# rising-turtle/graph_slam

Hardware: AMD Instinct MI355X
Metric: Gauss-Newton iterations/s + final chi2 rel-err, 100k-pose SE3 graph (higher is better)
Workload: dtype f64; 1 GPU; 100k-pose / 1.00M-edge synthetic Manhattan-3D SE3 pose graph, 1xMI355X; poses=100000, edges=999944, parallelism=single GPU

## Files before the change

### graph_slam_amd/__init__.py

```python
import ctypes as C
import os

import numpy as np

_HERE = os.path.dirname(os.path.abspath(__file__))
LIB_PATH = os.environ.get("FGO_LIB", os.path.join(_HERE, "libfgo.so"))

FGO_TANGENT_G2O = 0
FGO_TANGENT_GTSAM = 1


class FgoConfig(C.Structure):
    _fields_ = [("device", C.c_int), ("verbose", C.c_int), ("ordering", C.c_int), ("nd_leaf", C.c_int), ("order_candidates", C.c_int),
                ("reserved", C.c_int * 11)]


class FgoStats(C.Structure):
    _fields_ = [("iterations", C.c_int), ("trials", C.c_int), ("terminated", C.c_int), ("structure_rebuilt", C.c_int),
                ("chi2_initial", C.c_double), ("chi2_final", C.c_double), ("lambda_final", C.c_double),
                ("t_symbolic", C.c_double), ("t_upload", C.c_double), ("t_total", C.c_double),
                ("ms_linearize", C.c_double), ("ms_factor", C.c_double), ("ms_solve", C.c_double), ("ms_update", C.c_double),
                ("n_free", C.c_int64), ("n_edges", C.c_int64), ("nnz_H_blocks", C.c_int64), ("nnz_L_blocks", C.c_int64),
                ("n_update_ops", C.c_int64), ("n_levels", C.c_int), ("n_tasks", C.c_int),
                ("bytes_factor", C.c_double), ("bytes_linearize", C.c_double), ("bytes_solve", C.c_double),
# ... 159 lines not shown
class MapRenderView(C.Structure):
    _fields_ = [(f, C.c_int64) for f in ("n_valid", "n_drawn", "n_pixels", "n_meas", "n_both", "n_agree", "n_closer", "n_through")]


class MapRenderResult(C.Structure):
    _fields_ = [("n_points", C.c_int64), ("n_nonfinite", C.c_int64), ("form", C.c_int), ("tile_rows", C.c_int)]


FGO_MAP_RENDER_TILES, FGO_MAP_RENDER_GLOBAL = 0, 1


ALLREDUCE_FN = C.CFUNCTYPE(C.c_int, C.c_void_p, C.c_void_p, C.c_int64)


def _load():
    if not os.path.exists(LIB_PATH):
        raise ImportError(
            "graph_slam_amd: %s is missing — build it with `python -m graph_slam_amd.build` "
            "(hipcc, gfx950).  There is no CPU fallback." % LIB_PATH)
    lib = C.CDLL(LIB_PATH)
    dp, ip, i64p = C.POINTER(C.c_double), C.POINTER(C.c_int), C.POINTER(C.c_int64)
    lib.fgo_create.restype = C.c_void_p
    lib.fgo_create.argtypes = [C.POINTER(FgoConfig)]
    lib.fgo_destroy.argtypes = [C.c_void_p]
    lib.fgo_last_error.restype = C.c_char_p
    lib.fgo_last_error.argtypes = [C.c_void_p]
    lib.fgo_version.restype = C.c_char_p
    lib.fgo_device_count.restype = C.c_int
    lib.fgo_add_pose.argtypes = [C.c_void_p, C.c_int64, dp, dp, C.c_int]
    lib.fgo_set_pose.argtypes = [C.c_void_p, C.c_int64, dp, dp]
    lib.fgo_get_pose.argtypes = [C.c_void_p, C.c_int64, dp]
    lib.fgo_has_pose.argtypes = [C.c_void_p, C.c_int64]
    lib.fgo_num_poses.restype = C.c_int64
    lib.fgo_num_poses.argtypes = [C.c_void_p]
    lib.fgo_num_edges.restype = C.c_int64
    lib.fgo_num_edges.argtypes = [C.c_void_p]
    lib.fgo_add_poses.argtypes = [C.c_void_p, C.c_int64, i64p, dp, C.POINTER(C.c_ubyte)]
    lib.fgo_get_poses.argtypes = [C.c_void_p, C.c_int64, i64p, dp]
    lib.fgo_add_edge_se3.argtypes = [C.c_void_p, C.c_int64, C.c_int64, dp, dp, dp, C.c_int]
    lib.fgo_add_edges_se3.argtypes = [C.c_void_p, C.c_int64, i64p, i64p, dp, dp, C.c_int]
    lib.fgo_optimize.argtypes = [C.c_void_p, C.c_int, C.POINTER(FgoStats)]
    lib.fgo_chi2.restype = C.c_double
    lib.fgo_chi2.argtypes = [C.c_void_p]
    lib.fgo_trace.argtypes = [C.c_void_p, dp, dp, C.c_int]
    lib.fgo_linearize.argtypes = [C.c_void_p, dp, dp, dp, i64p]
    lib.fgo_solve_step.argtypes = [C.c_void_p, C.c_double, dp]
    lib.fgo_bench_phase.argtypes = [C.c_void_p, C.c_int, C.c_int, dp]
    lib.fgo_get_stats.argtypes = [C.c_void_p, C.POINTER(FgoStats)]
    lib.fgo_synth_manhattan3d.restype = C.c_int64
    lib.fgo_synth_manhattan3d.argtypes = [C.c_int64, C.c_int, C.c_int, C.c_uint64, C.c_double, C.c_double,
                                          dp, dp, i64p, i64p, dp, dp, C.c_int64]
    lib.fgo_shard_range.argtypes = [C.c_int64, C.c_int, C.c_int, i64p, i64p]
    lib.fgo_add_prior_pose.argtypes = [C.c_void_p, C.c_int64, dp, dp, dp]
    lib.fgo_optimize_gtsam.argtypes = [C.c_void_p, C.c_int, C.POINTER(FgoStats)]
    lib.fgo_error.restype = C.c_double
    lib.fgo_isam2_update.argtypes = [C.c_void_p, C.c_double, C.POINTER(FgoStats)]
    lib.fgo_isam2_reset.argtypes = [C.c_void_p]
    lib.fgo_isam2_get_state.argtypes = [C.c_void_p, C.c_int64, dp, dp]
    lib.fgo_error.argtypes = [C.c_void_p]
    lib.fgo_marginal_cov.argtypes = [C.c_void_p, C.c_int64, dp]
    lib.fgo_set_shard.argtypes = [C.c_void_p, C.c_int, C.c_int]
    lib.fgo_set_allreduce.argtypes = [C.c_void_p, ALLREDUCE_FN, C.c_void_p]
    lib.fgo_isam2_reserve.argtypes = [C.c_void_p, C.c_int, C.c_int]
    lib.fgo_set_growth.argtypes = [C.c_void_p, C.c_int, C.c_int]
    lib.fgo_isam2_set_wildfire.argtypes = [C.c_void_p, C.c_double]
    lib.fgo_marginal_cov_many.argtypes = [C.c_void_p, C.c_int64, i64p, dp]
    lib.fgo_marginal_cov_all.restype = C.c_int64
    lib.fgo_marginal_cov_all.argtypes = [C.c_void_p, C.c_int64, i64p, dp]
    lib.fgo_marginal_cov_pairs.argtypes = [C.c_void_p, C.c_int64, i64p, i64p, dp]
    lib.fgo_debug_selinv_stats.argtypes = [C.c_void_p, dp]
    lib.fgo_debug_selinv_census.argtypes = [C.c_void_p, i64p]
    lib.fgo_gate_edges_se3.argtypes = [C.c_void_p, C.c_int64, i64p, i64p, dp, dp, C.c_int, dp, dp, dp]
    lib.fgo_edge_chi2_se3.argtypes = [C.c_void_p, C.c_int64, C.c_int64, dp]
    lib.fgo_debug_gate_stats.argtypes = [C.c_void_p, dp]
    lib.fgo_gate_plane_factors.argtypes = [C.c_void_p, C.c_int64, i64p, i64p, dp, dp, dp, dp, dp, dp, dp]
    lib.fgo_associate_planes.argtypes = [C.c_void_p, C.c_int64, C.c_int64, dp, dp, C.c_int64, i64p, C.c_double, C.c_double, i64p, dp, dp]
    lib.fgo_dist_unique_id.argtypes = [C.c_void_p]
    lib.fgo_dist_init_rccl.argtypes = [C.c_void_p, C.c_void_p]
    lib.fgo_debug_partition.argtypes = [C.c_int, C.c_int64, C.POINTER(C.c_int), C.POINTER(C.c_int), C.c_int, C.POINTER(C.c_int)]
    lib.fgo_debug_allreduce.argtypes = [C.c_void_p, dp, C.c_int64]
    lib.fgo_debug_read_system.argtypes = [C.c_void_p, dp, dp, dp]
    lib.fgo_debug_read_reduced.argtypes = [C.c_void_p, C.c_double, dp, dp, i64p]
    lib.fgo_debug_solve_fused.argtypes = [C.c_void_p, C.c_double, dp]
    lib.fgo_debug_launch_census.argtypes = [C.c_void_p, C.c_int, i64p, i64p, i64p, C.c_int, C.POINTER(C.c_int), C.POINTER(C.c_int), C.c_int,
                                            C.POINTER(C.c_int), C.c_char_p, C.c_int]
    lib.fgo_debug_isam_last.argtypes = [C.c_void_p] + [C.POINTER(C.c_int)] * 6 + [C.c_int,
                                        C.POINTER(C.c_int), C.c_char_p, C.c_char_p, C.c_int, C.POINTER(C.c_int), C.c_char_p, dp, C.c_int64]
    lib.fgo_debug_linearize_census.argtypes = [C.c_void_p, i64p]
    lib.fgo_imu_params_vn100.argtypes = [dp]
    lib.fgo_preint_reset.argtypes = [dp, dp]
    lib.fgo_preint_integrate.argtypes = [dp, dp, dp, dp, C.c_double]
    lib.fgo_preint_predict.argtypes = [dp] * 7
    lib.fgo_set_fixed.argtypes = [C.c_void_p, C.c_int64, C.c_int]
    lib.fgo_preint_information.argtypes = [dp, dp]
    lib.fgo_preint_batch.argtypes = [C.c_int, C.c_int64, C.POINTER(C.c_int64), dp, dp, C.c_double, dp, dp, dp]
    lib.fgo_two_view_params_default.restype = None
    lib.fgo_two_view_params_default.argtypes = [C.POINTER(TwoViewParams)]
    lib.fgo_two_view_ba_batch.argtypes = [C.c_int, C.c_int64, i64p, dp, dp, dp, dp, dp, dp, C.POINTER(TwoViewParams), dp, dp, dp, dp,
                                          C.POINTER(TwoViewResult)]
    lib.fgo_plane_check_params_default.restype = None
    lib.fgo_plane_check_params_default.argtypes = [C.POINTER(PlaneCheckParams)]
    lib.fgo_plane_check_vro_batch.argtypes = [C.c_int, C.c_int64, dp, dp, dp, i64p, dp, dp, i64p, dp, dp, C.POINTER(PlaneCheckParams),
                                              C.POINTER(PlaneCheckResult), i64p, dp, dp, dp, dp, dp]
    lib.fgo_chi2_quantile.restype = C.c_double
    lib.fgo_chi2_quantile.argtypes = [C.c_int, C.c_double]
    lib.fgo_imu_check_params_default.restype = None
    lib.fgo_imu_check_params_default.argtypes = [C.POINTER(ImuCheckParams)]
    lib.fgo_imu_check_vro_batch.argtypes = [C.c_int, C.c_int64, dp, dp, dp, C.c_int64, dp, i64p, dp, dp, C.POINTER(ImuCheckParams),
                                            C.POINTER(ImuCheckResult), dp, dp]
    lib.fgo_vro_params_default.restype = None
    lib.fgo_vro_params_default.argtypes = [C.POINTER(VroParams)]
    lib.fgo_vro_ransac_batch.argtypes = [C.c_int, C.c_int64, i64p, dp, dp, C.POINTER(VroParams), dp, dp, dp, C.POINTER(C.c_ubyte),
                                         C.POINTER(C.c_int32), C.POINTER(VroResult)]
    lib.fgo_debug_vro_waves.argtypes = [C.c_int]
    lib.fgo_debug_vro_kernel_ms.restype = C.c_double
    lib.fgo_debug_vro_kernel_ms.argtypes = []
    lib.fgo_plane_extract_params_default.restype = None
    lib.fgo_plane_extract_params_default.argtypes = [C.POINTER(PlaneExtractParams)]
    lib.fgo_plane_extract_batch.argtypes = [C.c_int, C.c_int64, C.c_int, C.c_int, C.POINTER(C.c_uint16), C.POINTER(PlaneExtractParams),
                                            C.POINTER(PlaneExtractResult), dp, dp, dp, C.POINTER(PlaneExtractPlane),
                                            C.POINTER(C.c_int8), C.POINTER(C.c_int32)]
    lib.fgo_debug_plane_extract_kernel_ms.restype = C.c_double
    lib.fgo_debug_plane_extract_kernel_ms.argtypes = []
    lib.fgo_plane_propagate_params_default.restype = None
    lib.fgo_plane_propagate_params_default.argtypes = [C.POINTER(PlanePropagateParams)]
    lib.fgo_plane_propagate_batch.argtypes = [C.c_int, C.c_int64, C.c_int, C.c_int, C.POINTER(C.c_uint16), C.POINTER(C.c_uint8),
                                              C.POINTER(C.c_int8), C.POINTER(C.c_int32), dp, dp, C.c_int64, i64p, i64p, dp, dp, dp,
                                              C.POINTER(PlanePropagateParams), C.POINTER(PlanePropagateResult), dp, dp, dp,
                                              C.POINTER(PlanePropagatePlane), C.POINTER(PlanePropagatePred), C.POINTER(C.c_int8)]
    lib.fgo_debug_plane_propagate_kernel_ms.restype = C.c_double
    lib.fgo_debug_plane_propagate_kernel_ms.argtypes = []
    lib.fgo_match_params_default.restype = None
    lib.fgo_match_params_default.argtypes = [C.POINTER(MatchParams)]
    i32p, u8p = C.POINTER(C.c_int32), C.POINTER(C.c_uint8)
    lib.fgo_match_features_batch.argtypes = [C.c_int, C.c_int64, i64p, u8p, dp, dp, C.c_int64, i64p, i64p, dp, u8p, C.POINTER(MatchParams),
                                             C.POINTER(MatchResult), i64p, i32p, i32p, i32p, u8p, i64p, i64p, i64p, dp, dp, dp, dp, i32p]
    lib.fgo_debug_match_kernel_ms.restype = C.c_double
    lib.fgo_debug_match_kernel_ms.argtypes = []
    lib.fgo_map_params_default.restype = None
    lib.fgo_map_params_default.argtypes = [C.POINTER(MapParams)]
    lib.fgo_map_fuse_batch.argtypes = [C.c_int, C.c_int64, C.c_int, C.c_int, C.POINTER(C.c_uint16), u8p, C.c_int, dp, dp, C.POINTER(MapParams),
                                       C.c_int64, C.POINTER(MapResult), dp, u8p, C.POINTER(C.c_int32), i64p, i64p, dp]
    lib.fgo_debug_map_fuse_kernel_ms.restype = C.c_double
    lib.fgo_debug_map_fuse_kernel_ms.argtypes = []
    lib.fgo_map_clean_params_default.restype = None
    lib.fgo_map_clean_params_default.argtypes = [C.POINTER(MapCleanParams)]
    lib.fgo_map_clean.argtypes = [C.c_int, C.c_int64, dp, C.POINTER(MapCleanParams), C.POINTER(MapCleanResult), C.POINTER(C.c_int32), u8p,
                                  C.POINTER(C.c_int32), i64p, dp]
    lib.fgo_debug_map_clean_kernel_ms.restype = C.c_double
    lib.fgo_debug_map_clean_kernel_ms.argtypes = []
    lib.fgo_map_normals_params_default.restype = None
    lib.fgo_map_normals_params_default.argtypes = [C.POINTER(MapNormalsParams)]
    lib.fgo_map_normals.argtypes = [C.c_int, C.c_int64, dp, C.POINTER(MapNormalsParams), C.POINTER(MapNormalsResult), dp, dp, dp, i32p, u8p,
                                    i32p, i64p, i64p]
    lib.fgo_debug_map_normals_kernel_ms.restype = C.c_double
    lib.fgo_debug_map_normals_kernel_ms.argtypes = []
    lib.fgo_map_render_params_default.restype = None
    lib.fgo_map_render_params_default.argtypes = [C.POINTER(MapRenderParams)]
    lib.fgo_map_render_batch.argtypes = [C.c_int, C.c_int64, dp, u8p, C.c_int, C.c_int64, dp, dp, dp, C.c_int, C.c_int,
                                         C.POINTER(MapRenderParams), C.POINTER(C.c_uint16), C.POINTER(MapRenderResult),
                                         C.POINTER(MapRenderView), i32p, i32p, u8p, dp]
    lib.fgo_debug_map_render_kernel_ms.restype = C.c_double
    lib.fgo_debug_map_render_kernel_ms.argtypes = []
    lib.fgo_add_vec3.argtypes = [C.c_void_p, C.c_int64, dp]
    lib.fgo_add_bias.argtypes = [C.c_void_p, C.c_int64, dp]
    lib.fgo_add_prior_vec3.argtypes = [C.c_void_p, C.c_int64, dp, C.c_double]
# ... 1047 lines not shown
        z = np.ascontiguousarray(z_abcd, np.float64); s = np.ascontiguousarray(cov_ut6, np.float64)
        self._chk(lib.fgo_add_plane_factor(self._h, pose_id, plane_id, _dp(z), _dp(s)))

    def add_point(self, pid, xyz):
        a = np.ascontiguousarray(xyz, np.float64)
        self._chk(lib.fgo_add_point3(self._h, pid, _dp(a)))

    def add_prior_point(self, pid, xyz, sigma):
        a = np.ascontiguousarray(xyz, np.float64)
        self._chk(lib.fgo_add_prior_point3(self._h, pid, _dp(a), sigma))

    def set_calibration(self, calib9, body_P_sensor7=None):
        c9 = [float(x) for x in calib9]
        b = None if body_P_sensor7 is None else _dp(np.ascontiguousarray(body_P_sensor7, np.float64))
        self._chk(lib.fgo_set_calib_ds2(self._h, *c9, b))

    def add_reproj(self, pose_id, point_id, uv, sigma=1.0):
        a = np.ascontiguousarray(uv, np.float64)
        self._chk(lib.fgo_add_reproj(self._h, pose_id, point_id, _dp(a), sigma))

    def optimize_gtsam(self, max_iters=100):
        st = FgoStats()
        rc = self._chk(lib.fgo_optimize_gtsam(self._h, max_iters, C.byref(st)))
        return rc, st

    def isam2_update(self, relinearize_threshold=0.1):
        st = FgoStats()
        self._chk(lib.fgo_isam2_update(self._h, relinearize_threshold, C.byref(st)))
        return st

    def isam2_set_wildfire(self, threshold):
        self._chk(lib.fgo_isam2_set_wildfire(self._h, threshold))

    def isam2_reserve(self, reserve_variables, window=0):
        self._chk(lib.fgo_isam2_reserve(self._h, reserve_variables, window))

    def set_growth(self, reserve_variables, window=0):
        self._chk(lib.fgo_set_growth(self._h, reserve_variables, window))

    def isam2_reset(self):
        self._chk(lib.fgo_isam2_reset(self._h))

    def isam2_state(self, pid):
        th = np.zeros(7); de = np.zeros(6)
        self._chk(lib.fgo_isam2_get_state(self._h, pid, _dp(th), _dp(de)))
        return th, de

    def error(self):
        v = lib.fgo_error(self._h)
        if v != v:
            raise FgoError("fgo_error failed: %s" % lib.fgo_last_error(self._h).decode())
        return v

    def trace(self, cap=256):
        a = np.zeros(cap); b = np.zeros(cap)
        m = self._chk(lib.fgo_trace(self._h, _dp(a), _dp(b), cap))
        return a[:m], b[:m]

    def linearize(self, dense=True):
        chi = C.c_double(); nf = C.c_int64()
        if not dense:
            self._chk(lib.fgo_linearize(self._h, C.byref(chi), None, None, C.byref(nf)))
            return chi.value, None, None
        self._chk(lib.fgo_linearize(self._h, C.byref(chi), None, None, C.byref(nf)))
        m = 6 * nf.value
        H = np.zeros((m, m)); b = np.zeros(m)
        self._chk(lib.fgo_linearize(self._h, C.byref(chi), _dp(H), _dp(b), C.byref(nf)))
        return chi.value, H, b

    def solve_step(self, lam):
        chi = C.c_double(); nf = C.c_int64()
        self._chk(lib.fgo_linearize(self._h, C.byref(chi), None, None, C.byref(nf)))
        d = np.zeros(6 * nf.value)
        self._chk(lib.fgo_solve_step(self._h, lam, _dp(d)))
        return d

    def solve_fused(self, lam):
        chi = C.c_double(); nf = C.c_int64()
        self._chk(lib.fgo_linearize(self._h, C.byref(chi), None, None, C.byref(nf)))
        d = np.zeros(6 * nf.value)
        self._chk(lib.fgo_debug_solve_fused(self._h, lam, _dp(d)))
        return d

    def launch_census(self, fused=True):
        ip = C.POINTER(C.c_int)
        names = C.create_string_buffer(4096)
        n = self._chk(lib.fgo_debug_launch_census(self._h, int(fused), None, None, None, 0, None, None, 0, None, names, len(names)))
        nl = int(self.stats().n_levels)
        la = np.zeros(n, np.int64); wg = np.zeros(n, np.int64); it = np.zeros(n, np.int64)
        lr = np.zeros(max(nl, 1), np.int32); ll = np.zeros(max(nl, 1), np.int32); ch = np.zeros(2, np.int32)
        self._chk(lib.fgo_debug_launch_census(self._h, int(fused), _i64p(la), _i64p(wg), _i64p(it), n, lr.ctypes.data_as(ip), ll.ctypes.data_as(ip), nl,
                                              ch.ctypes.data_as(ip), None, 0))
        keys = names.value.decode().split("\n")[:n]
        return dict(forms={k: (int(a), int(w), int(i)) for k, a, w, i in zip(keys, la, wg, it)}, level_riders=[int(v) for v in lr[:nl]],
                    level_long=[int(v) for v in ll[:nl]], chain_on=bool(ch[0]), chain_mode=int(ch[1]))

    def isam2_last(self):
        ip = C.POINTER(C.c_int)
        info = np.zeros(5, np.int32)
        n = self._chk(lib.fgo_debug_isam_last(self._h, info.ctypes.data_as(ip), None, None, None, None, None, 0, None, None, None, 0, None, None, None, 0))
        nl, nt = int(info[2]), int(info[3])
        lo = np.zeros(max(nl, 1), np.int32); hi = np.zeros(max(nl, 1), np.int32); cnt = np.zeros(max(nl, 1), np.int32)
        fw = np.zeros(max(nl, 1), np.int32); ft = np.zeros(max(nl, 1), np.int32)
        tl = np.zeros(max(nt, 1), np.int32); td = np.zeros(max(nt, 1), np.uint8); tr = np.zeros(max(nt, 1), np.uint8)
        vt = np.zeros(max(n, 1), np.int32); vc = np.zeros(max(n, 1), np.uint8); de = np.zeros((max(n, 1), 6))
        cp = lambda a: a.ctypes.data_as(C.c_char_p)
        self._chk(lib.fgo_debug_isam_last(self._h, info.ctypes.data_as(ip), lo.ctypes.data_as(ip), hi.ctypes.data_as(ip), cnt.ctypes.data_as(ip),
                                          fw.ctypes.data_as(ip), ft.ctypes.data_as(ip), nl,
                                          tl.ctypes.data_as(ip), cp(td), cp(tr), nt, vt.ctypes.data_as(ip), cp(vc), _dp(de), n))
        return dict(sweep=int(info[0]), cut=bool(info[1]), chain_low=int(info[4]), level_lo=lo[:nl], level_hi=hi[:nl], level_ntask=cnt[:nl], level_fwd=fw[:nl], level_fwtab=ft[:nl], task_level=tl[:nt],
                    task_dirty=td[:nt], task_run=tr[:nt], var_task=vt[:n], var_chg=vc[:n], delta=de[:n])

    LINEARIZE_CENSUS = ("n_hubs", "n_hub_vars", "n_hub_multi", "hub_deg", "hub_cap", "n_dup_groups", "n_dup_members", "n_priors",
                        "n_phantom", "imu_ncolor", "maskable", "structure_rebuilt")

    def linearize_census(self):
        out = np.zeros(12, np.int64)
        self._chk(lib.fgo_debug_linearize_census(self._h, _i64p(out)))
        return {k: int(v) for k, v in zip(self.LINEARIZE_CENSUS, out)}

    def bench_phase(self, phase, reps):
        ms = C.c_double()
        self._chk(lib.fgo_bench_phase(self._h, phase, reps, C.byref(ms)))
        return ms.value

    def stats(self):
        st = FgoStats()
        self._chk(lib.fgo_get_stats(self._h, C.byref(st)))
        return st
```

### graph_slam_amd/csrc/device_plan.hpp

```cpp
#pragma once
#include <hip/hip_runtime.h>
#include <stdint.h>
#include <vector>
#include "fgo_internal.hpp"

namespace fgo {

struct CamCalib {
  double fx, fy, s, u0, v0, k1, k2, p1, p2;
  double bps[7];
  double ad[36];
};
bool cam_calib_make(CamCalib &K, const double calib9[9], const double *body_P_sensor7);

struct ImuPayload {
  double dt;
  double dR[4];
  double dp[3], dv[3];
  double J_R_bg[9], J_p_ba[9], J_p_bg[9], J_v_ba[9], J_v_bg[9];
  double bhat[6];
  double info[225];
  double pad;
};
static_assert(sizeof(ImuPayload) == 288 * sizeof(double), "ImuPayload layout");

struct AccDesc { int t, a; long long o0, o1; };
struct LeafDesc { int task, c_begin, m, k0; long long base, obase; int nblk, nops; };
struct PanelDesc { int task, m, cols0, prow0, nrows, chunk0, nchunks, top; };
struct RowChunk { int pn, m, s0, R6, prow0, cols0, top, task; };
struct BwdChunk { int pn, m, row0, nrows; };
struct ChainItem { int pn, need; };

constexpr int NJMAX = (6 * PANEL_MAX + 15) / 16;
constexpr int NLT = NJMAX * (NJMAX - 1) / 2;
constexpr int NTILE = NLT + NJMAX;
constexpr int PTOP_TILE = 256;
static_assert(NTILE == NJMAX * (NJMAX + 1) / 2, "ptop: one slot per tile of the lower triangle, diagonal included");

struct PanelPlan {
  const PanelDesc *pdesc;
  const LeafDesc *leaf_desc, *leaf_lpt;
  const int *tri_order;
  const RowChunk *rchunks;
  const BwdChunk *bchunks;
  const ChainItem *bchain;
  unsigned *bchain_done;
  const int *task_panel, *panel_task;
  const int *ptri_blk;
  const int *prow_ptr, *prow_idx, *prow_blk;
  const int *pchunk_panel, *pchunk_row0, *pchunk_nrows, *panel_chunk0;
  const int64_t *row_mid;
  const int *fchunk_col;
  const int64_t *fchunk_e0;
  const int *pcol_fchunk0, *pcol_fchunkn;
  const int *rchunk_panel, *rchunk_s0;
  const int *rchunk_src;
  int rchunk_src0;
  const int *ptri_src, *prow_src;
  double *ptop;
  double *fpart;
  double *bpart;
};

struct RideItem;

constexpr int EDGE_REC = 32;
constexpr int HUB_DEG = 1024;
constexpr int HUB_SLICE = 512, HUB_MAX_SLICES = 64, HUB_MAX_VARS = 1024, HUB_PART = 42;

struct BaPlan {
  int n_lm;
  const unsigned char *lm_mine;
  int64_t n_obs;
  int n_tgt, n_cam;
  const int *lm_var;
  const int64_t *pt_ptr;
  const int *pt_obs;
  const double *pt_uvw;
  const int *pt_cam;
  const int64_t *lp_ptr;
  const double *lp_val;
  const double *obs_uvw;
  const int *obs_cam;
  const int *obs_col;
  const int *obs_lm;
  const int64_t *cam_ptr;
  const int *cam_col;
  int64_t o_first;
  int n_tgt_small;
  const int *tgt_list;
  int n_tgt_list;
  const int64_t *cam_t0;
  const int *cam_list;
  int n_cam_list;
  const int *tgt_blk;
  const int64_t *tgt_ptr;
  const int *op_a, *op_b;
  const int *op_lm;
  double *pt_val;
  double *Hinv, *zp;
};

struct DevPlan {
  PanelPlan pp;
  int64_t n_poses, n_edges;
  int64_t n_real;
  int64_t edge_stride;
  int64_t n_imu;
  const ImuPayload *imu;
  const int *imu_ids;
  const int *imu_slot;
  int64_t imu_fn;
  const int *imu_list;
  int imu_ncolor;
  const int *imu_color_ptr_h;
  double *imu_stash;
  double gravity[3];
  const int *var_kind;
  const int *edge_kind;
  CamCalib cam;
  int nb;
  int64_t n_hblocks;
  int lin_priors;
  int zero_offdiag;
  const int *pose_col;
  const int *edge_i, *edge_j;
  const double *ainv;
  const double *info;
  const int *edge_slot;
  const int *hub_list;
  const int *hub_slice;
  int n_hubs;
  int hub_deg;
  double *hub_part;
  const int *hubm;
  int n_hub_multi;
  const int64_t *he_ptr;
  const int *he;
  int64_t n_dup_groups;
  const int64_t *dup_ptr;
  const int64_t *dup_edges;
  const int *dup_slot;
  int64_t n_priors;
  const int64_t *prior_ptr;
  const int *prior_pose;
  const double *prior_minv;
  const double *prior_info;
  const int64_t *colptr;
  const int *rowidx;
  const int *asrc;
  int prof_tri;
  int zero_blk;
  const int64_t *op_ptr;
  const int64_t *op_mid;
  const int *op_a, *op_b;
  const int *acc_targets;
  const AccDesc *acc_desc;
  const int *g2_tgt;
  const int64_t *g2_ptr;
  const int *g2_b;
  const int *g2_a;
  const unsigned char *task_dirty;
  const int *acc_task;
  const int *g2_task;
  const int *tcol_task;
  BaPlan ba;
  const int *fwg_ci, *fwg_ch;
  const int *fwd_f0, *fwd_fn;
  const int *fsplit_ci;
  const RideItem *ride_items;
  int ride_xcd;
  const int64_t *acc_start;
  const int64_t *rowptr;
  const int *row_blk, *row_col;
  const int *task_ptr, *task_cols;
  double *partial;
  int dist;
  int top_col0;
  int64_t top_blk0;
  const int64_t *top_ext0;
  const int64_t *own_op0, *own_op1;
  const int64_t *top_row0;
  const int64_t *own_row0, *own_row1;
  const unsigned char *var_mine;
  int lambda_rank;
};

struct HostSchedule {
  int cus = 256;
  int n_levels = 0;
  int world = 1, rank = 0;
  std::vector<int> seg_group;
  int64_t n_top_blocks = 0;
  int n_top_cols = 0;
  std::vector<int> level_ptr;
  std::vector<int64_t> acc_ptr, acc_mid;
  std::vector<int> ride_ptr;
  std::vector<int64_t> g2_lvl;
  std::vector<int> level_maxcol;
  std::vector<int> level_maxrow;
  std::vector<int> level_maxtaskcols;
  std::vector<char> level_leaf;
  std::vector<int> level_leaf_maxblk, level_leaf_maxops;
  std::vector<char> level_panel;
  int rows_byc_level = 1 << 30;
  std::vector<int> level_pn0;
  std::vector<int> level_col_ptr;
  std::vector<int> fwg_ptr;
  std::vector<int> fsplit_ptr;
  std::vector<int> pchunk_ptr, fchunk_ptr, rchunk_ptr;
  int bchain_low = -1, bchain_n = 0;
};

void launch_linearize(const DevPlan &P, const double *poses, double *Hblk, double *bvec, double *scalar_out, hipStream_t s);
void launch_chi2(const DevPlan &P, const double *poses, double *scalar_out, hipStream_t s);
void launch_maxdiag(const DevPlan &P, const double *Hblk, double *scalar_out, hipStream_t s);
void launch_update(const DevPlan &P, const double *poses, double *cand, const double *x, const double *b,
                   const double *lambda_p, double *scalar_out, hipStream_t s);
enum { PHASE_ALL = 0, PHASE_DOMAIN = 1, PHASE_TOP = 2 };
struct PartialSweep {
  const int *t_lo, *t_hi;
  const int64_t *s0, *s1, *l0, *l1;
  const int *g0, *g1, *c0, *c1;
  const int *task_ptr;
};
enum LaunchForm {
  LF_ACC8 = 0, LF_ACC4, LF_ACC2, LF_ACC1,
  LF_ACC2_8, LF_ACC2_4, LF_ACC2_1,
  LF_FWD_COMBINE,
  LF_TRI16, LF_TRI8, LF_TRI1,
  LF_ROWS, LF_ROWS_BYC,
  LF_LEAF4,
  LF_FACT_1_2, LF_FACT_1_3, LF_FACT_4_3, LF_FACT_8_3, LF_FACT_16_2,
  LF_FWD1, LF_FWD4, LF_FWD16,
  LF_FWD_EXT, LF_FWD_TRI,
  LF_BWD_CHAIN, LF_BWD_FUSED, LF_BWD_EXT, LF_BWD_TRI,
  LF_BWD1, LF_BWD4, LF_BWD8,
  LF_COUNT
};
const char *launch_form_name(int form);
struct LaunchCensus {
  int64_t launches[LF_COUNT] = {}, workgroups[LF_COUNT] = {};
  int64_t items[LF_COUNT] = {};
  std::vector<int> level_riders, level_long;
  std::vector<int> level_fwd, level_fwtab;
  int chain_on = 0, chain_mode = 0;
  void add(int form, int64_t grid, int64_t n_items = -1) { ++launches[form]; workgroups[form] += grid; items[form] += n_items < 0 ? grid : n_items; }
};
LaunchForm select_acc(const HostSchedule &H, int l);
LaunchForm select_tri(const HostSchedule &H, int l);
LaunchForm select_rows(const HostSchedule &H, int l);
LaunchForm select_fact(const HostSchedule &H, int l);
LaunchForm select_fwd(const HostSchedule &H, int l);
LaunchForm select_bwd(const HostSchedule &H, int l);
void launch_factor(const DevPlan &P, const HostSchedule &H, const double *Hblk, double *Lv, const double *lambda_p,
                   int *fail_flag, hipStream_t s, const double *b = nullptr, double *x = nullptr, int phase = PHASE_ALL, const PartialSweep *ps = nullptr,
                   const double *b_full = nullptr, LaunchCensus *census = nullptr);
struct Wildfire { unsigned char *run, *chg; const unsigned char *dirty; const double *xprev; double thr; };
void launch_solve(const DevPlan &P, const HostSchedule &H, const double *Lv, const double *b, double *x, hipStream_t s,
                  bool fwd_done = false, int phase = PHASE_ALL, const Wildfire *wf = nullptr, LaunchCensus *census = nullptr);
void launch_mix_rhs(const DevPlan &P, const double *b, const double *ysaved, double *x, const unsigned char *col_dirty, hipStream_t s);
void launch_copy_vec(const double *src, double *dst, int64_t n, hipStream_t s);
void launch_mask_poses(const DevPlan &P, const double *poses, double *out, const int *pose_group, int rank, int world, hipStream_t s);
int linearize_blocks(const DevPlan &P);
void launch_reduce(const double *partial, int64_t n, double *out, int mode, hipStream_t s);
void prepare_device_kernels();
void launch_zero(double *p, int64_t n, hipStream_t s);
void launch_zero_flag(int *p, hipStream_t s);
void launch_pack_scalars(double *scal, const int *fail, hipStream_t s, double *host = nullptr);
void launch_fetch_scalar(double *dst, const double *src_host, hipStream_t s);
void launch_scatter_edges(const double *stage, int64_t n, int64_t e0, double *rec, hipStream_t s);
bool linearize_gtsam_maskable(const DevPlan &P);
void launch_linearize_gtsam_masked(const DevPlan &P, const double *poses, double *Hblk, double *bvec, double *scalar_out, hipStream_t s,
                                   const unsigned char *mask, double *chi_var);
void launch_linearize_gtsam(const DevPlan &P, const double *poses, double *Hblk, double *bvec, double *scalar_out, hipStream_t s,
                            double *ba_W = nullptr, double *ba_Hpp = nullptr, double *ba_bp = nullptr);
int ba_linearize_blocks(const DevPlan &P);
void launch_ba_linearize(const DevPlan &P, const double *vals, double *W, double *Hpp, double *bp, double *Hblk, double *bvec, double *chi_partial, hipStream_t s);
void launch_ba_reduce(const DevPlan &P, const double *W, const double *Hpp, const double *bp, const double *H, const double *b,
                      double *Hred, double *bred, const double *lambda_p, int *fail_flag, hipStream_t s);
void launch_ba_back(const DevPlan &P, const double *W, const double *bp, double *x, hipStream_t s);
void launch_chi2_gtsam(const DevPlan &P, const double *poses, double *scalar_out, hipStream_t s);
void launch_update_gtsam(const DevPlan &P, const double *poses, double *cand, const double *x, const double *b,
                         const double *lambda_p, double *scalar_out, hipStream_t s);
void launch_isam2_relin(const DevPlan &P, double *theta, double *delta, double thr, double *count_out, hipStream_t s, unsigned char *moved_out = nullptr);
void launch_isam2_estimate(const DevPlan &P, const double *theta, const double *x, double *delta, double *est, hipStream_t s,
                           unsigned char *moved_next = nullptr, double thr_next = 0);

struct SinvPlan {
  int nb;
  const int64_t *colptr;
  const int *task_ptr, *task_cols;
  const int64_t *sptr;
  const int *sidx;
  const double *U;
  double *Sig;
};
void launch_sinv_prep(const SinvPlan &Q, const double *Lv, double *U, hipStream_t s);
void launch_sinv_sweep(const SinvPlan &Q, const HostSchedule &H, hipStream_t s);
void launch_sinv_gather(const int64_t *enc, int64_t n, const double *Sig, double *out, hipStream_t s);
void launch_sinv_rows(const int *cols, int64_t n, const double *x, double *out, hipStream_t s, int64_t istride = 6, int64_t rstride = 1);

constexpr int64_t GATE_ZERO = -1, GATE_EXTRA0 = -2;
inline int64_t gate_extra_code(int64_t slot, bool transpose) { return GATE_EXTRA0 - ((slot << 1) | (transpose ? 1 : 0)); }
constexpr int GATE_REC = 28;
struct GatePlan {
  int64_t n;
  const int *va, *vb;
  const double *rec;
  const int64_t *enc;
  const double *Sig, *extra;
  double *out;
  int want_P;
};
void launch_gate(const GatePlan &A, const double *values, bool gtsam, bool with_cov, hipStream_t s);

constexpr int PGATE_REC = 10;
struct PlaneGatePlan {
  int64_t n;
  const int *vx, *vp;
  const double *rec;
  const int64_t *enc;
  const double *Sig, *extra;
  double *out;
  int want_P;
};
void launch_plane_gate(const PlaneGatePlan &A, const double *values, hipStream_t s);
void launch_plane_assoc(const double *gate_out, int64_t k, int64_t m, double d2_gate, double cos_min, bool want_matrix, double *res, hipStream_t s);

}
```

### graph_slam_amd/csrc/fgo_ctx.hpp

```cpp
#pragma once
#include <hip/hip_runtime.h>
#include <algorithm>
#include <atomic>
#include <chrono>
#include <cmath>
#include <cstdio>
#include <cstdlib>
#include <cstring>
#include <limits>
#include <map>
#include <mutex>
#include <new>
#include <stdexcept>
#include <string>
#include <unordered_map>
#include <vector>
#include "../../include/fgo.h"
#include "device_plan.hpp"
#include "fgo_internal.hpp"
#include "rccl_min.hpp"

namespace fgo {

template <class T>
struct DevBuf {
  T *p = nullptr;
  size_t n = 0, cap = 0;
  ~DevBuf() { release(); }
  void release() { if (p) { (void)hipFree(p); p = nullptr; n = 0; cap = 0; } }
  hipError_t alloc(size_t count) {
    if (p && count <= cap) { n = count; return hipSuccess; }
    const bool regrow = p != nullptr;
    release();
    cap = (count ? count : 1) + (regrow ? count / 4 : 0);
    const hipError_t e = hipMalloc((void **)&p, sizeof(T) * cap);
    if (e != hipSuccess) { p = nullptr; cap = 0; return e; }
    n = count;
    return hipSuccess;
  }
  template <class A>
  hipError_t upload(const std::vector<T, A> &h, hipStream_t s) {
    hipError_t e = alloc(h.size());
    if (e != hipSuccess) return e;
    if (h.empty()) return hipSuccess;
    return hipMemcpyAsync(p, h.data(), sizeof(T) * h.size(), hipMemcpyHostToDevice, s);
  }
  void swap(DevBuf &o) { std::swap(p, o.p); std::swap(n, o.n); std::swap(cap, o.cap); }
};

enum class LHolds { scratch, undamped, undamped_sigma, isam_step };

}

struct fgo_ctx {
  fgo_config cfg{};
  std::string err;
  std::unordered_map<int64_t, int> id2idx;
  std::vector<int64_t> ids;
  std::vector<double> poses;
  std::vector<unsigned char> fixed;
  std::vector<int> ei, ej;
  std::vector<double> meas, info;
  std::vector<int> torder;
  std::vector<int> prior_v;
  std::vector<double> prior_mean, prior_info;
  bool gtsam_mode = false;
  bool structure_dirty = true;
  bool host_poses_newer = true;
  bool dev_poses_newer = false;
  bool lin_valid = false;
  hipStream_t stream = nullptr;
  bool use_graph = true;
  fgo::Symbolic S;
  fgo::HostSchedule sched;
  fgo::DevPlan plan{};
  int64_t n_offdiag = 0;
  fgo::DevBuf<int> d_pose_col, d_edge_i, d_edge_j, d_edge_slot, d_he, d_dup_slot, d_rowidx, d_asrc, d_op_a, d_op_b,
      d_acc_targets, d_row_blk, d_row_col, d_task_ptr, d_task_cols, d_fail;
  fgo::DevBuf<int64_t> d_he_ptr, d_dup_ptr, d_dup_edges, d_colptr, d_op_ptr, d_op_mid, d_rowptr, d_g2_ptr;
  fgo::DevBuf<int> d_g2_tgt, d_g2_b, d_g2_a;
  fgo::DevBuf<fgo::RideItem> d_ride_items;
  fgo::DevBuf<int> d_fwg_ci, d_fwg_ch, d_fwd_f0, d_fwd_fn, d_fsplit_ci;
  fgo::DevBuf<int64_t> d_acc_start;
  fgo::DevBuf<double> d_ainv, d_partial, d_poses[2], d_H[2], d_b[2], d_x, d_L, d_scal;
  struct BaSchur {
    bool on = false;
    int n_lm = 0;
    fgo::DevBuf<unsigned char> d_lm_mine;
    fgo::DevBuf<int> d_lm_var, d_pt_obs, d_tgt_list, d_obs_cam, d_obs_col, d_obs_lm, d_cam_col, d_tgt_blk, d_op_a, d_op_b, d_op_lm, d_pt_cam;
    fgo::DevBuf<int64_t> d_pt_ptr, d_cam_ptr, d_tgt_ptr, d_lp_ptr, d_cam_t0;
    fgo::DevBuf<int> d_cam_list;
    fgo::DevBuf<double> d_obs_uvw, d_pt_uvw, d_lp_val, d_W[2], d_Hpp[2], d_bp[2], d_Hinv, d_zp, d_pt_val, d_Hred, d_bred;
  } ba;
  bool ba_disable = false;
  fgo::DevBuf<int> d_task_panel, d_panel_task, d_ptri_blk, d_prow_ptr, d_prow_idx, d_prow_blk, d_pchunk_panel, d_pchunk_row0,
      d_pchunk_nrows, d_panel_chunk0, d_fchunk_col, d_pcol_fchunk0, d_pcol_fchunkn;
  fgo::DevBuf<int64_t> d_row_mid, d_fchunk_e0;
  fgo::DevBuf<double> d_fpart, d_bpart, d_ptop, d_imu_stash;
  fgo::DevBuf<int> d_rchunk_panel, d_rchunk_s0, d_ptri_src, d_prow_src;
  fgo::DevBuf<int> d_hub_list, d_hub_slice, d_hubm;
  fgo::DevBuf<double> d_hub_part;
  fgo::DevBuf<fgo::PanelDesc> d_pdesc;
  fgo::DevBuf<int> d_tri_order, d_rchunk_src;
  fgo::DevBuf<fgo::LeafDesc> d_leaf_desc, d_leaf_lpt;
  fgo::DevBuf<fgo::AccDesc> d_acc_desc;
  fgo::DevBuf<fgo::RowChunk> d_rchunks;
  fgo::DevBuf<fgo::BwdChunk> d_bchunks;
  fgo::DevBuf<fgo::ChainItem> d_bchain;
  fgo::DevBuf<unsigned> d_bchain_done;
  fgo::DevBuf<int64_t> d_prior_ptr;
  fgo::DevBuf<int> d_prior_pose, d_var_kind, d_edge_kind;
  std::vector<int> var_kind;
  fgo::CamCalib cam{};
  bool cam_set = false;
  std::vector<int> imu_ids;
  std::vector<fgo::ImuPayload> imu_payload;
  double gravity[3] = {0.0, 0.0, 9.71};
  int shard_rank = 0, shard_world = 1;
  fgo_allreduce_fn ar_fn = nullptr;
  void *ar_user = nullptr;
  ncclComm_t rccl = nullptr;
  std::vector<int> pose_group;
  fgo::DevBuf<int> d_pose_group, d_imu_list;
  fgo::DevBuf<int64_t> d_top_ext0, d_own_op0, d_own_op1, d_top_row0, d_own_row0, d_own_row1;
  fgo::DevBuf<unsigned char> d_var_mine;
  fgo::DevBuf<double> d_status;
  fgo::DevBuf<double> d_gather;
  hipGraphExec_t dist_graph[2][2] = {{nullptr, nullptr}, {nullptr, nullptr}};
  double xgmi_bytes = 0;
  fgo::DevBuf<fgo::ImuPayload> d_imu;
  fgo::DevBuf<int> d_imu_ids, d_imu_slot;
  fgo::DevBuf<double> d_prior_minv, d_prior_info;
  int cur = 0;
  fgo::LHolds L_holds = fgo::LHolds::scratch;
  std::vector<int> h_pose_col;
  struct SelInv {
    bool lists = false;
    fgo::DevBuf<int64_t> d_sptr, d_enc;
    fgo::DevBuf<int> d_sidx;
    fgo::DevBuf<double> d_U, d_Sig, d_out;
    double t_build = 0, ms_factor = 0, ms_prep = 0, ms_sweep = 0;
    int64_t n_entries = 0, list_bytes = 0;
    int64_t n_fallback = 0;
    void release() {
      lists = false;
      d_sptr.release(); d_enc.release(); d_sidx.release(); d_U.release(); d_Sig.release(); d_out.release();
    }
  } sinv;
  struct Gate {
    fgo::DevBuf<int> d_v, d_cols;
    fgo::DevBuf<int64_t> d_enc;
    fgo::DevBuf<double> d_rec, d_extra, d_out, d_rhs, d_res;
    int64_t n_off = 0, n_groups = 0;
    double ms_kernel = 0, ms_solves = 0;
  } gate;
  fgo::DevBuf<double> d_theta, d_delta;
  int64_t isam_E_seen = 0, isam_NI_seen = 0, isam_NP_seen = 0;
  std::vector<int> col_task;
  fgo::DevBuf<double> d_y;
  fgo::DevBuf<unsigned char> d_moved, d_task_dirty, d_col_dirty, d_moved_next;
  unsigned char *h_flags = nullptr;
  fgo::DevBuf<unsigned char> d_lin_mask;
  fgo::DevBuf<double> d_chi_var;
  bool isam_H_valid = false;
  std::vector<int> isam_set_tasks, isam_set_cols;
  std::vector<int64_t> isam_set_aff;
  std::vector<int64_t> tk_s0, tk_s1, tk_l0, tk_l1;
  std::vector<int> tk_g0, tk_g1, tk_c0, tk_c1, task_level, lvl_lo, lvl_hi;
  bool tk_ok = false;
  int isam_last_sweep = 0;
  bool isam_last_cut = false;
  fgo::PartialSweep partial_sweep() const {
    return fgo::PartialSweep{lvl_lo.data(), lvl_hi.data(), tk_s0.data(), tk_s1.data(), tk_l0.data(), tk_l1.data(),
                             tk_g0.data(), tk_g1.data(), tk_c0.data(), tk_c1.data(), S.task_ptr.data()};
  }
  double wild_thr = 0;
  bool wild_valid = false;
  fgo::DevBuf<double> d_xprev;
  fgo::DevBuf<unsigned char> d_bwd_run, d_chg;
  bool isam_moved_valid = false;
  double isam_moved_thr = -1;
  int64_t isam_moved_nx = 0;
  size_t h_flags_cap = 0;
  fgo::DevBuf<int> d_acc_task, d_g2_task, d_tcol_task;
  int64_t isam_n = 0;
  bool isam_incremental = false;
// ... 101 lines not shown
```

### graph_slam_amd/csrc/fgo_inspect.cpp

```cpp
#include "fgo_ctx.hpp"

using namespace fgo;

extern "C" {

int fgo_debug_read_system(fgo_ctx *c, double *H, double *b, double *chi2) try {
  if (!c) return FGO_EINVAL;
  (void)hipSetDevice(c->cfg.device);
  ba_off(c);
  int rc = ensure_ready(c);
  if (rc) return rc;
  if (c->n_phantom > 0) return fail(c, FGO_ESTATE, "fgo_debug_read_system: the structure carries the growth reserve of the incremental mode (fgo_isam2_reset drops it)");
  hipStream_t s = c->stream;
  if (c->gtsam_mode) launch_linearize_gtsam(c->plan, c->d_poses[c->cur].p, c->d_H[c->cur].p, c->d_b[c->cur].p, c->d_scal.p + 0, s);
  else launch_linearize(c->plan, c->d_poses[c->cur].p, c->d_H[c->cur].p, c->d_b[c->cur].p, c->d_scal.p + 0, s);
  c->lin_valid = false;
  drop_undamped(c);
  if (H) HIPCHK(c, hipMemcpyAsync(H, c->d_H[c->cur].p, sizeof(double) * 36 * (size_t)c->plan.n_hblocks, hipMemcpyDeviceToHost, s));
  if (b) HIPCHK(c, hipMemcpyAsync(b, c->d_b[c->cur].p, sizeof(double) * 6 * (size_t)c->plan.nb, hipMemcpyDeviceToHost, s));
  if (chi2) HIPCHK(c, hipMemcpyAsync(chi2, c->d_scal.p, sizeof(double), hipMemcpyDeviceToHost, s));
  HIPCHK(c, hipStreamSynchronize(s));
  HIPCHK(c, hipGetLastError());
  return FGO_OK;
} FGO_CATCH_INT(c)
// ... 31 lines not shown
  HIPCHK(c, hipMemcpy(b.data(), db, sizeof(double) * b.size(), hipMemcpyDeviceToHost));
  HIPCHK(c, hipMemcpy(asrc.data(), c->d_asrc.p, sizeof(int) * asrc.size(), hipMemcpyDeviceToHost));
  const size_t m = (size_t)nreal * 6;
  if (H_dense) {
    std::memset(H_dense, 0, sizeof(double) * m * m);
    for (int k = 0; k < nb; ++k)
      for (int64_t t = c->S.colptr[k]; t < c->S.colptr[k + 1]; ++t) {
        if (asrc[t] < 0) continue;
        const int hr = c->S.perm[c->S.rowidx[t]], hc = c->S.perm[k];
        if (hr >= nreal || hc >= nreal) continue;
        const double *B = &H[(size_t)asrc[t] * 36];
        for (int r = 0; r < 6; ++r)
          for (int q = 0; q < 6; ++q) {
            H_dense[((size_t)hr * 6 + r) * m + (size_t)hc * 6 + q] = B[r * 6 + q];
            H_dense[((size_t)hc * 6 + q) * m + (size_t)hr * 6 + r] = B[r * 6 + q];
          }
      }
  }
  if (b_dense)
    for (int k = 0; k < nb; ++k) if (c->S.perm[k] < nreal) std::memcpy(b_dense + (size_t)c->S.perm[k] * 6, &b[(size_t)k * 6], 6 * sizeof(double));
  return FGO_OK;
}

int fgo_linearize(fgo_ctx *c, double *chi2_out, double *H_dense, double *b_dense, int64_t *n_free_out) try {
  if (!c) return FGO_EINVAL;
  (void)hipSetDevice(c->cfg.device);
  if (H_dense || b_dense) ba_off(c);
  int rc = ensure_ready(c);
  if (rc) return rc;
  rc = linearize_current(c, false);
  if (rc) return rc;
  if (chi2_out) *chi2_out = c->chi_cur;
  if (n_free_out) *n_free_out = (int64_t)c->plan.nb - c->n_phantom + (c->ba.on ? c->ba.n_lm : 0);
  if (!H_dense && !b_dense) return FGO_OK;
  return dense_from_blocks(c, c->d_H[c->cur].p, c->d_b[c->cur].p, H_dense, b_dense);
} FGO_CATCH_INT(c)

int fgo_debug_read_reduced(fgo_ctx *c, double lambda, double *H_dense, double *b_dense, int64_t *n_out) try {
  if (!c || !(lambda >= 0)) return FGO_EINVAL;
  (void)hipSetDevice(c->cfg.device);
  int rc = ensure_ready(c);
  if (rc) return rc;
  if (!c->ba.on) return fail(c, FGO_ESTATE, "fgo_debug_read_reduced: no landmarks are eliminated in this structure");
  rc = linearize_current(c, false);
  if (rc) return rc;
  if (n_out) *n_out = (int64_t)c->plan.nb - c->n_phantom;
  if (!H_dense && !b_dense) return FGO_OK;
  hipStream_t s = c->stream;
  HIPCHK(c, stage_lambda(c, lambda));
  launch_ba_reduce(c->plan, c->ba.d_W[c->cur].p, c->ba.d_Hpp[c->cur].p, c->ba.d_bp[c->cur].p, c->d_H[c->cur].p, c->d_b[c->cur].p,
                   c->ba.d_Hred.p, c->ba.d_bred.p, c->d_scal.p + 3, c->d_fail.p, s);
  HIPCHK(c, hipStreamSynchronize(s));
  HIPCHK(c, hipGetLastError());
  return dense_from_blocks(c, c->ba.d_Hred.p, c->ba.d_bred.p, H_dense, b_dense);
} FGO_CATCH_INT(c)

static int solve_once(fgo_ctx *c, double lambda, double *delta_out, bool fused, const char *who) {
  if (!c || !delta_out) return FGO_EINVAL;
  if (c->shard_world > 1) return fail(c, FGO_ESTATE, (std::string(who) + ": not available in distributed mode").c_str());
  (void)hipSetDevice(c->cfg.device);
  ba_off(c);
  int rc = ensure_ready(c);
  if (rc) return rc;
  if (!c->lin_valid) { rc = linearize_current(c, false); if (rc) return rc; }
  hipStream_t s = c->stream;
  claim_L(c);
  HIPCHK(c, stage_lambda(c, lambda));
  launch_factor(c->plan, c->sched, c->d_H[c->cur].p, c->d_L.p, c->d_scal.p + 3, c->d_fail.p, s, fused ? c->d_b[c->cur].p : nullptr, fused ? c->d_x.p : nullptr);
  launch_solve(c->plan, c->sched, c->d_L.p, c->d_b[c->cur].p, c->d_x.p, s, fused);
  const int nb = c->plan.nb;
  std::vector<double> x((size_t)nb * 6);
  HIPCHK(c, hipMemcpyAsync(x.data(), c->d_x.p, sizeof(double) * x.size(), hipMemcpyDeviceToHost, s));
  HIPCHK(c, hipMemcpyAsync(c->h_fail, c->d_fail.p, sizeof(int), hipMemcpyDeviceToHost, s));
  HIPCHK(c, hipStreamSynchronize(s));
  HIPCHK(c, hipGetLastError());
  for (int k = 0; k < nb; ++k)
    if (c->S.perm[k] < nb - c->n_phantom) std::memcpy(delta_out + (size_t)c->S.perm[k] * 6, &x[(size_t)k * 6], 6 * sizeof(double));
  if (*c->h_fail) return fail(c, FGO_ENUM, "block Cholesky: matrix not positive definite");
  return FGO_OK;
}
int fgo_solve_step(fgo_ctx *c, double lambda, double *delta_out) try { return solve_once(c, lambda, delta_out, false, "fgo_solve_step"); } FGO_CATCH_INT(c)
int fgo_debug_solve_fused(fgo_ctx *c, double lambda, double *delta_out) try { return solve_once(c, lambda, delta_out, true, "fgo_debug_solve_fused"); } FGO_CATCH_INT(c)

int fgo_debug_launch_census(fgo_ctx *c, int fused, int64_t *launches, int64_t *workgroups, int64_t *items, int form_cap, int *level_riders, int *level_long,
                            int level_cap, int *chain2, char *names, int names_cap) try {
  if (!c || form_cap < 0 || level_cap < 0 || names_cap < 0) return FGO_EINVAL;
  if (c->shard_world > 1) return fail(c, FGO_ESTATE, "fgo_debug_launch_census: not available in distributed mode");
  (void)hipSetDevice(c->cfg.device);
  if (fused != 2) ba_off(c);
  if (fused == 2 && (c->structure_dirty || c->isam_last_sweep == 0 || c->col_task.empty()))
    return fail(c, FGO_ESTATE, "fgo_debug_launch_census: the last fgo_isam2_update on this structure was not a partial sweep");
  int rc = ensure_ready(c);
  if (rc) return rc;
  LaunchCensus cz;
  double *const b = c->d_b[c->cur].p, *const x = c->d_x.p;
  if (!b || !x) return fail(c, FGO_ESTATE, "fgo_debug_launch_census: the right-hand side / solution buffers are not allocated");
  DevPlan plan = c->plan;
  PartialSweep ps{};
  if (fused == 2) { plan.task_dirty = c->d_task_dirty.p; if (c->isam_last_sweep == 2) ps = c->partial_sweep(); }
  launch_factor(plan, c->sched, c->d_H[c->cur].p, c->d_L.p, c->d_scal.p + 3, c->d_fail.p, c->stream, fused ? b : nullptr, fused ? x : nullptr, PHASE_ALL,
                fused == 2 && c->isam_last_sweep == 2 ? &ps : nullptr, nullptr, &cz);
  launch_solve(c->plan, c->sched, c->d_L.p, b, x, c->stream, fused != 0, PHASE_ALL, nullptr, &cz);
  for (int f = 0; f < std::min<int>(form_cap, LF_COUNT); ++f) {
    if (launches) launches[f] = cz.launches[f];
    if (workgroups) workgroups[f] = cz.workgroups[f];
    if (items) items[f] = cz.items[f];
  }
  for (int l = 0; l < std::min(level_cap, c->sched.n_levels); ++l) {
    if (level_riders) level_riders[l] = cz.level_riders[(size_t)l];
    if (level_long) level_long[l] = cz.level_long[(size_t)l];
  }
  if (chain2) { chain2[0] = cz.chain_on; chain2[1] = cz.chain_mode; }
  if (names && names_cap > 0) {
    std::string all;
    for (int f = 0; f < LF_COUNT; ++f) { all += launch_form_name(f); all += '\n'; }
    if ((int)all.size() + 1 > names_cap) return fail(c, FGO_EINVAL, "fgo_debug_launch_census: names buffer too small");
    std::memcpy(names, all.c_str(), all.size() + 1);
  }
  return LF_COUNT;
} FGO_CATCH_INT(c)

int fgo_debug_linearize_census(fgo_ctx *c, int64_t out[12]) try {
  if (!c || !out) return FGO_EINVAL;
  (void)hipSetDevice(c->cfg.device);
  int rc = ensure_ready(c);
  if (rc) return rc;
  const DevPlan &P = c->plan;
  out[0] = P.n_hubs; out[1] = c->n_hub_vars; out[2] = P.n_hub_multi; out[3] = P.hub_deg; out[4] = (int64_t)c->hub_entry_cap;
  out[5] = P.n_dup_groups; out[6] = c->n_dup_members;
  out[7] = P.n_priors; out[8] = c->n_phantom; out[9] = P.imu_ncolor;
  out[10] = c->gtsam_mode && linearize_gtsam_maskable(P) ? 1 : 0;
  out[11] = c->last_phase_rebuilt;
  return FGO_OK;
} FGO_CATCH_INT(c)

int fgo_debug_isam_last(fgo_ctx *c, int *info5, int *level_lo, int *level_hi, int *level_ntask, int *level_fwd, int *level_fwtab, int level_cap, int *task_level, unsigned char *task_dirty,
                        unsigned char *task_run, int task_cap, int *var_task, unsigned char *var_chg, double *var_delta, int64_t var_cap) try {
  if (!c || level_cap < 0 || task_cap < 0 || var_cap < 0) return FGO_EINVAL;
  (void)hipSetDevice(c->cfg.device);
  if (c->structure_dirty || c->col_task.empty() || !c->inc.valid || c->isam_n <= 0)
    return fail(c, FGO_ESTATE, "fgo_debug_isam_last: no fgo_isam2_update has run on the current structure");
  const int nl = c->sched.n_levels, ntask = (int)c->S.task_ptr.size() - 1, nb = c->plan.nb;
  const int64_t N = c->isam_n;
  if (info5) { info5[0] = c->isam_last_sweep; info5[1] = c->isam_last_cut ? 1 : 0; info5[2] = nl; info5[3] = ntask; info5[4] = c->sched.bchain_low; }
  const bool ranged = c->isam_last_sweep == 2;
  for (int l = 0; l < std::min(level_cap, nl); ++l) {
    if (level_lo) level_lo[l] = ranged ? c->lvl_lo[(size_t)l] : c->sched.level_ptr[l];
    if (level_hi) level_hi[l] = ranged ? c->lvl_hi[(size_t)l] : c->sched.level_ptr[l + 1] - 1;
    if (level_ntask) level_ntask[l] = c->sched.level_ptr[l + 1] - c->sched.level_ptr[l];
  }
  if ((level_fwd || level_fwtab) && level_cap > 0) {
    LaunchCensus cz;
    DevPlan plan = c->plan;
    PartialSweep ps{};
    if (c->isam_last_sweep != 0) plan.task_dirty = c->d_task_dirty.p;
    if (ranged) ps = c->partial_sweep();
    launch_factor(plan, c->sched, c->d_H[c->cur].p, c->d_L.p, c->d_scal.p + 3, c->d_fail.p, c->stream, c->d_b[c->cur].p, c->d_x.p, PHASE_ALL,
                  ranged ? &ps : nullptr, nullptr, &cz);
    for (int l = 0; l < std::min(level_cap, nl); ++l) {
      if (level_fwd) level_fwd[l] = cz.level_fwd[(size_t)l];
      if (level_fwtab) level_fwtab[l] = cz.level_fwtab[(size_t)l];
    }
  }
  const int nt = std::min(task_cap, ntask);
  if (task_level) for (int t = 0; t < nt; ++t) task_level[t] = c->task_level[(size_t)t];
  if (task_dirty) {
// ... 53 lines not shown
```

### graph_slam_amd/csrc/fgo_internal.hpp

```cpp
#pragma once
#include <cstdint>
#include <cstdlib>
#include <exception>
#include <thread>
#include <pthread.h>
#include <mutex>
#include <condition_variable>
#include <functional>
#include <atomic>
#include <algorithm>
#include <memory>
#include <string>
#include <unordered_map>
#include <vector>

namespace fgo {

template <class T>
struct NoInitAlloc : std::allocator<T> {
  template <class U> struct rebind { typedef NoInitAlloc<U> other; };
  NoInitAlloc() = default;
  template <class U> NoInitAlloc(const NoInitAlloc<U> &) {}
  template <class U> void construct(U *p) { ::new ((void *)p) U; }
  template <class U, class... A> void construct(U *p, A &&...a) { ::new ((void *)p) U(std::forward<A>(a)...); }
};
typedef std::vector<int, NoInitAlloc<int>> IntList;

inline int host_threads() {
  static const int nthreads = [] {
    const char *e = std::getenv("FGO_HOST_THREADS");
    int t = e ? std::atoi(e) : (int)std::min(32u, std::max(1u, std::thread::hardware_concurrency()));
    return std::max(1, t);
  }();
  return nthreads;
}
inline double tune(const char *key, double dflt) {
  static const std::unordered_map<std::string, double> *tab = [] {
    auto *m = new std::unordered_map<std::string, double>();
    if (const char *e = std::getenv("FGO_TUNE")) {
      std::string s(e);
      size_t i = 0;
      while (i < s.size()) {
        size_t j = s.find(',', i);
        if (j == std::string::npos) j = s.size();
        const std::string kv = s.substr(i, j - i);
        const size_t q = kv.find('=');
        if (q != std::string::npos && q > 0) (*m)[kv.substr(0, q)] = std::atof(kv.c_str() + q + 1);
        i = j + 1;
      }
    }
    return m;
  }();
  const auto it = tab->find(key);
  return it == tab->end() ? dflt : it->second;
}
class HostPool {
 public:
  static HostPool &get() {
    static std::once_flag once;
    std::call_once(once, [] { pthread_atfork(nullptr, nullptr, [] { instance().store(nullptr); }); });
    HostPool *p = instance().load();
    if (!p) {
      HostPool *fresh = new HostPool;
      if (instance().compare_exchange_strong(p, fresh)) p = fresh; else delete fresh;
    }
    return *p;
  }
  template <class F>
  bool run(int nworkers, F &&job) {
    std::unique_lock<std::mutex> own(busy_, std::try_to_lock);
    if (!own.owns_lock()) return false;
    ensure(nworkers);
    std::exception_ptr err;
    std::mutex err_m;
    auto guarded = [&](int w) {
      try { job(w); }
      catch (...) { std::lock_guard<std::mutex> g(err_m); if (!err) err = std::current_exception(); }
    };
    {
      std::lock_guard<std::mutex> lk(m_);
      job_ = guarded;
      active_ = std::min(nworkers, (int)th_.size());
      pending_ = active_;
      ++epoch_;
    }
    cv_.notify_all();
    guarded(-1);
    {
      std::unique_lock<std::mutex> lk(m_);
      done_.wait(lk, [&] { return pending_ == 0; });
      job_ = nullptr;
    }
    if (err) std::rethrow_exception(err);
    return true;
  }
 private:
  static std::atomic<HostPool *> &instance() { static std::atomic<HostPool *> p{nullptr}; return p; }
  void ensure(int n) {
    while ((int)th_.size() < n) {
      const int id = (int)th_.size();
      uint64_t seen;
      { std::lock_guard<std::mutex> lk(m_); seen = epoch_; }
      th_.emplace_back([this, id, seen]() mutable {
        for (;;) {
          std::function<void(int)> job;
          {
            std::unique_lock<std::mutex> lk(m_);
            cv_.wait(lk, [&] { return epoch_ != seen; });
            seen = epoch_;
            if (id >= active_) continue;
            job = job_;
          }
          job(id);
          { std::lock_guard<std::mutex> lk(m_); if (--pending_ == 0) done_.notify_all(); }
        }
      });
    }
  }
  std::mutex busy_, m_;
  std::condition_variable cv_, done_;
  std::vector<std::thread> th_;
  std::function<void(int)> job_;
  int active_ = 0, pending_ = 0;
  uint64_t epoch_ = 0;
};
template <class F>
inline void parallel_ranges(int n, int chunk, F &&fn) {
  const int nthreads = host_threads();
  const int nchunks = (n + chunk - 1) / chunk;
  const int nt = std::min(nthreads, nchunks);
  if (nt <= 1) { if (n > 0) fn(0, n); return; }
  std::atomic<int> next{0};
  auto worker = [&](int) {
    for (int c = next.fetch_add(1); c < nchunks; c = next.fetch_add(1)) fn(c * chunk, std::min(n, (c + 1) * chunk));
  };
  if (!HostPool::get().run(nt - 1, worker)) worker(-1);
}

// ... 97 lines not shown
```

### graph_slam_amd/csrc/kernels_factor.hip

```cpp
#include <hip/hip_runtime.h>
#include <mutex>
#include <vector>
#include <stdint.h>
#include "device_plan.hpp"
#include "fgo_internal.hpp"
#include "sweep_device.hpp"

namespace fgo {

typedef double d4_t __attribute__((ext_vector_type(4)));

__device__ __forceinline__ void row_update(Row6 &acc, const Row6 &a, const double *__restrict__ B) {
#pragma unroll
  for (int c = 0; c < 6; ++c) {
    const Row6 b = load_row(B + 6 * c);
    acc.v[c] -= a.v[0] * b.v[0] + a.v[1] * b.v[1] + a.v[2] * b.v[2] + a.v[3] * b.v[3] + a.v[4] * b.v[4] + a.v[5] * b.v[5];
  }
}
__device__ __forceinline__ Row6 load_A_row(const DevPlan &P, const double *__restrict__ Hblk, int64_t t, int r, double lambda) {
  const int a = P.asrc[t];
  Row6 x = {{0, 0, 0, 0, 0, 0}};
  if (a >= 0) {
    x = load_row(Hblk + 36 * (int64_t)a + 6 * r);
    if (a < P.nb) {
// ... 410 lines not shown
      if (q == b0) {
#pragma unroll
        for (int rr = 0; rr < 6; ++rr)
          if (rr == r) {
#pragma unroll
            for (int c = 0; c < 6; ++c) lq.v[c] = (c <= rr) ? Lk[rr * (rr + 1) / 2 + c] : 0.0;
          }
        if (x) {
#pragma unroll
          for (int rr = 0; rr < 6; ++rr) if (rr == r) yr[6 * ci + rr] = yk[rr];
        }
      } else {
        lq = trsm_row(load_row(Ls + 36 * q + 6 * r), Lk, invd);
        if (x) {
          const int i2 = lrow[q];
          if (i2 != 0xffff)
            xr[6 * i2 + r] -= lq.v[0] * yk[0] + lq.v[1] * yk[1] + lq.v[2] * yk[2] + lq.v[3] * yk[3] + lq.v[4] * yk[4] + lq.v[5] * yk[5];
        }
      }
      store_row(Ls + 36 * q + 6 * r, lq);
    }
    __syncthreads();
  }
  if (x) for (int i = threadIdx.x; i < 6 * m; i += NW * 64) x[6 * (int64_t)k0 + i] = yr[i];
  double2 *__restrict__ dst = reinterpret_cast<double2 *>(Lv + 36 * base);
  const double2 *__restrict__ src = reinterpret_cast<const double2 *>(Ls);
  for (int i = threadIdx.x; i < nblk * 18; i += NW * 64) dst[i] = src[i];
}

struct PairTab { unsigned char a[PM * (PM + 1) / 2], b[PM * (PM + 1) / 2]; };
constexpr PairTab make_pairs() {
  PairTab t{};
  int q = 0;
  for (int a = 0; a < PM; ++a)
    for (int b = 0; b <= a; ++b) { t.a[q] = (unsigned char)a; t.b[q] = (unsigned char)b; ++q; }
  return t;
}
__constant__ PairTab PAIRS = make_pairs();
#define PAIR_A PAIRS.a
#define PAIR_B PAIRS.b
#define TRI(rr, kk) ((((rr) * ((rr) + 1)) / 2 + (kk)) * 36)

template <bool FROM_LDS>
__device__ __forceinline__ Row6 trsm_row_blk(const Row6 &u, const double *__restrict__ L) {
  Row6 x;
#pragma unroll
  for (int c = 0; c < 6; ++c) {
    double s = u.v[c];
#pragma unroll
    for (int m = 0; m < 6; ++m) if (m < c) s -= x.v[m] * L[6 * c + m];
    x.v[c] = s / L[7 * c];
  }
  return x;
}

__device__ __forceinline__ void ride_items16(const DevPlan &P, const double *__restrict__ Hblk, double *__restrict__ Lv,
                                             const double *__restrict__ lambda_p, int item0, int nitems, int wg, double *__restrict__ smem) {
  const int lane = threadIdx.x & 63, wave = threadIdx.x >> 6;
  const int g = lane / 6, r = lane - 6 * g;
  const int part = wave >> 2, w4 = wave & 3;
  const int ii = RIDE_PER_WG * wg + part;
  const bool have = ii < nitems;
  const RideItem it = P.ride_items[item0 + (have ? ii : 0)];
  const bool run = have && (!P.task_dirty || P.task_dirty[it.task]);
  double *__restrict__ tile = smem + 360 * wave;
  if (run && lane < 60) {
    const int gid = w4 * 10 + g;
    Row6 acc = {{0, 0, 0, 0, 0, 0}};
    if (gid == 0 && it.first != 2) acc = it.first ? load_A_row(P, Hblk, it.t, r, *lambda_p) : load_row(Lv + 36 * (int64_t)it.t + 6 * r);
    apply_ops(P, Lv, acc, g, r, it.o0 + gid, it.o0 + it.n, 40, tile);
#pragma unroll
    for (int c = 0; c < 6; ++c) tile[6 * lane + c] = acc.v[c];
  }
  __syncthreads();
  const int tl = (int)threadIdx.x - 256 * part;
  if (run && tl < 36) {
    const double *pf = smem + 1440 * part;
    double sum = 0;
    for (int q = 0; q < 40; ++q) sum += pf[q * 36 + tl];
    Lv[36 * (int64_t)it.t + tl] = it.first == 2 ? -sum : sum;
  }
}

template <int NW>
__global__ __launch_bounds__(NW * 64) void k_panel_tri(DevPlan P, const double *__restrict__ Hblk, double *__restrict__ Lv, int pn0,
                                                    const double *__restrict__ lambda_p, int *__restrict__ fail_flag, int n_pn, int ride0, int n_ride, int n_real) {
  __shared__ __attribute__((aligned(16))) double T[PM * (PM + 1) / 2 * 36];
  if (NW == 16) {
    __shared__ __attribute__((aligned(16))) double ride_smem[NW == 16 ? 16 * 360 : 2];
    if ((int)blockIdx.x >= n_pn) {
      const int nwg = (int)gridDim.x - n_pn;
      ride_items16(P, Hblk, Lv, lambda_p, ride0, n_ride, P.ride_xcd ? xcd_contiguous((int)blockIdx.x - n_pn, nwg) : (int)blockIdx.x - n_pn, ride_smem);
      return;
    }
  }
  const long long t_begin = __builtin_readcyclecounter();
  if ((int)blockIdx.x >= n_real) return;
  const int pn = (NW == 8 && !P.task_dirty) ? P.pp.tri_order[pn0 + blockIdx.x] : pn0 + (int)blockIdx.x;
  const PanelDesc dsc = P.pp.pdesc[pn];
  if (!task_runs(P, dsc.task)) return;
  const int m = dsc.m;
  const int64_t tri0 = (int64_t)pn * (PM * PM);
  const int *__restrict__ tb = P.pp.ptri_blk + tri0;
  const int lane = threadIdx.x & 63, wave = threadIdx.x >> 6;
  const int g = lane / 6, r = lane - 6 * g;
  const bool lane_on = lane < 60;
  const int gid = wave * 10 + g;
  const double lambda = *lambda_p;
  const int npair = m * (m + 1) / 2;
  for (int gq = gid; lane_on && gq < npair; gq += NW * 10) {
    const int rr = PAIR_A[gq], kk = PAIR_B[gq];
    const int sc = P.pp.ptri_src[tri0 + rr * PM + kk];
    const double *base = sc >= 0 ? Lv + 36 * (int64_t)sc : (sc <= -2 ? Hblk + 36 * (int64_t)(-2 - sc) : Lv + 36 * (int64_t)P.zero_blk);
    Row6 x = load_row(base + 6 * r);
    if (sc <= -2 && rr == kk) {
#pragma unroll
      for (int c = 0; c < 6; ++c) x.v[c] += (c == r) ? lambda : 0.0;
    }
    store_row(&T[36 * gq + 6 * r], x);
  }
  __syncthreads();
  const int n = 6 * m, nJ = (n + 15) >> 4;
  long long *__restrict__ stamp = (P.prof_tri && n_real == 1 && m == PM) ? reinterpret_cast<long long *>(P.partial) : nullptr;
  if (stamp && threadIdx.x == 0) { stamp[0] = t_begin; stamp[1] = __builtin_readcyclecounter(); }
  if (wave == 0) {
    constexpr int HMAX = (PM + 9) / 10;
    for (int k = 0; k < m; ++k) {
      if (stamp && lane == 0) stamp[8 + 5 * k] = __builtin_readcyclecounter();
      Row6 acc[HMAX];
#pragma unroll
      for (int h = 0; h < HMAX; ++h) {
        const int rr = k + g + 10 * h;
        if (lane_on && rr < m) {
          acc[h] = load_row(&T[TRI(rr, k) + 6 * r]);
          if (k > 0) {
            const Row6 a = load_row(&T[TRI(rr, k - 1) + 6 * r]);
            const double *__restrict__ B = &T[TRI(k, k - 1)];
#pragma unroll
            for (int j = 0; j < 6; ++j)
#pragma unroll
              for (int c = 0; c < 6; ++c) acc[h].v[c] = fma(-a.v[j], B[6 * c + j], acc[h].v[c]);
          }
        }
      }
      if (lane_on && g == 0) store_row(&T[TRI(k, k) + 6 * r], acc[0]);
      __builtin_amdgcn_wave_barrier();
      if (stamp && lane == 0) stamp[8 + 5 * k + 1] = __builtin_readcyclecounter();
      double Lk[21], invd[6];
      const bool ok = chol6_lds(&T[TRI(k, k)], Lk, invd);
      if (!ok && lane == 0) atomicOr(fail_flag, 1);
      __builtin_amdgcn_wave_barrier();
      if (stamp && lane == 0) stamp[8 + 5 * k + 2] = __builtin_readcyclecounter() + (long long)(Lk[0] == 12345.678);
#pragma unroll
      for (int h = 0; h < HMAX; ++h) {
        const int rr = k + g + 10 * h;
        if (lane_on && rr < m) {
          Row6 x = trsm_row(acc[h], Lk, invd);
          if (rr == k) {
#pragma unroll
            for (int c = 0; c < 6; ++c) x.v[c] = (c <= r) ? x.v[c] : 0.0;
          }
          store_row(&T[TRI(rr, k) + 6 * r], x);
        }
      }
      if (stamp && lane == 0) stamp[8 + 5 * k + 3] = __builtin_readcyclecounter();
      __syncthreads();
      if (stamp && lane == 0) stamp[8 + 5 * k + 4] = __builtin_readcyclecounter();
    }
  } else {
    const int nn = lane & 15, q4 = lane >> 4;
    const int ntile = nJ * (nJ + 1) / 2;
    constexpr bool EXCL = NW >= 16;
    constexpr int NWORK = EXCL ? NW - NW / 4 : NW - 1;
    constexpr int NT = (NJMAX * (NJMAX + 1) / 2 + NWORK - 1) / NWORK;
    const bool idle = EXCL && (wave & 3) == 0;
    const int aw = EXCL ? wave - 1 - (wave >> 2) : wave - 1;
    d4_t C[NT];
    bool own[NT];
    int offA[NT], rrA[NT], offB[NT], rrB[NT], cj[NT], offE[NT][4], rrE[NT][4], tI[NT];
#pragma unroll
    for (int u = 0; u < NT; ++u) {
      const int p = aw + NWORK * u;
      own[u] = !idle && p < ntile;
      const int I = PAIR_A[own[u] ? p : 0], K = PAIR_B[own[u] ? p : 0];
      tI[u] = I;
      const int iA = 16 * I + nn, iB = 16 * K + nn;
      rrA[u] = iA < n ? iA / 6 : -1; offA[u] = TRI(iA / 6, 0) + (iA % 6) * 6;
      rrB[u] = iB < n ? iB / 6 : -1; offB[u] = TRI(iB / 6, 0) + (iB % 6) * 6;
      cj[u] = iB % 6;
      C[u] = d4_t{0.0, 0.0, 0.0, 0.0};
#pragma unroll
      for (int r4 = 0; r4 < 4; ++r4) {
        const int i = 16 * I + q4 + 4 * r4;
        rrE[u][r4] = i < n ? i / 6 : -1; offE[u][r4] = TRI(i / 6, 0) + (i % 6) * 6;
        if (own[u] && rrE[u][r4] >= 0 && rrB[u] >= 0 && rrE[u][r4] >= rrB[u]) C[u][r4] = T[offE[u][r4] + 36 * rrB[u] + cj[u]];
      }
    }
    for (int k = 0; k < m; ++k) {
      if (k > 0) {
#pragma unroll
        for (int u = 0; u < NT; ++u)
          if (own[u] && 16 * tI[u] + 15 >= 6 * k) {
#pragma unroll
            for (int kc = 0; kc < 2; ++kc) {
              const int c = 4 * kc + q4;
              double a = 0.0, b = 0.0;
              if (c < 6) {
                if (rrA[u] > k - 1) a = -T[offA[u] + (k - 1) * 36 + c];
                if (rrB[u] > k - 1) b = T[offB[u] + (k - 1) * 36 + c];
              }
              C[u] = __builtin_amdgcn_mfma_f64_16x16x4f64(a, b, C[u], 0, 0, 0);
            }
          }
#pragma unroll
        for (int u = 0; u < NT; ++u)
          if (own[u] && rrB[u] == k + 1) {
#pragma unroll
            for (int r4 = 0; r4 < 4; ++r4)
              if (rrE[u][r4] >= k + 1) T[offE[u][r4] + (k + 1) * 36 + cj[u]] = C[u][r4];
          }
      }
      __syncthreads();
    }
  }
  if (stamp && threadIdx.x == 0) stamp[2] = __builtin_readcyclecounter();
  auto Ls = [&](int i, int j) -> double {
    if (i >= n || j >= n) return (i == j) ? 1.0 : 0.0;
    const int rr = i / 6, kk = j / 6;
    if (rr < kk) return 0.0;
    return T[TRI(rr, kk) + (i - 6 * rr) * 6 + (j - 6 * kk)];
  };
  double *__restrict__ tp = P.pp.ptop + (int64_t)dsc.top * 256;
  __shared__ double Dt[NJMAX * 256];
  __shared__ double Dr[NW >= 16 ? NJMAX * 16 : 1];
  auto copy_out = [&](int gq0, int gstep, int e0, int estep) {
    for (int gq = gq0; lane_on && gq < npair; gq += gstep) {
      const int rr = PAIR_A[gq], kk = PAIR_B[gq];
      const int t = tb[rr * PM + kk];
      if (t >= 0) store_row(Lv + 36 * (int64_t)t + 6 * r, load_row(&T[36 * gq + 6 * r]));
    }
    for (int e = e0; e < (nJ * (nJ - 1) / 2) * 256; e += estep) {
      const int tile = e >> 8, kc = (e >> 6) & 3, l = e & 63;
      const int J = PAIR_A[tile] + 1, I = PAIR_B[tile];
      tp[e] = -Ls(16 * J + (l & 15), 16 * I + 4 * kc + (l >> 4));
    }
  };
  auto invert = [&]() {
    if ((int)threadIdx.x < 16 * nJ) {
      const int J = threadIdx.x >> 4, c = threadIdx.x & 15;
      double xc[16];
      const double *__restrict__ D = &Dt[J * 256];
      if (NW >= 16) {
        Dr[threadIdx.x] = 1.0 / D[c * 17];
        __builtin_amdgcn_wave_barrier();
      }
#pragma unroll
      for (int i = 0; i < 16; ++i) xc[i] = (i == c) ? 1.0 : 0.0;
#pragma unroll
      for (int i = 0; i < 16; ++i) {
        xc[i] *= NW >= 16 ? Dr[16 * J + i] : 1.0 / D[i * 17];
#pragma unroll
        for (int i2 = 0; i2 < 16; ++i2) if (i2 > i) xc[i2] = fma(-D[i2 * 16 + i], xc[i], xc[i2]);
      }
#pragma unroll
      for (int i = 0; i < 16; ++i) tp[(NLT + J) * 256 + 16 * c + i] = xc[i];
    }
  };
  if (NW < 16) copy_out(gid, NW * 10, (int)threadIdx.x, NW * 64);
  for (int e = threadIdx.x; e < nJ * 256; e += NW * 64) Dt[e] = Ls(16 * (e >> 8) + ((e >> 4) & 15), 16 * (e >> 8) + (e & 15));
  __syncthreads();
  if (NW < 16 || wave < 2) invert();
  else copy_out(gid - 20, (NW - 2) * 10, (int)threadIdx.x - 128, (NW - 2) * 64);
  if (stamp && threadIdx.x == 0) { stamp[3] = __builtin_readcyclecounter(); stamp[4] = wall_clock64(); }
}

constexpr int tri1_tile(int I, int K) { return I * (I + 1) / 2 + K; }
constexpr int TRI1_NR = 16 * NJMAX;
struct Tri1Ctx {
  const double *Hblk; double *Lv; double *tp; int64_t zero_blk;
  int m, n, nJ, lane, nn, q;
  double lambda;
  int rr[2], rho[2];
  bool rv[2], rpad[2];
};
__device__ __forceinline__ const double *tri1_src_row(const Tri1Ctx &X, const int *__restrict__ tsrc, int h, int k) {
  const int sc = tsrc[X.rr[h] * PM + k];
  const double *base = sc >= 0 ? X.Lv + 36 * (int64_t)sc : (sc <= -2 ? X.Hblk + 36 * (int64_t)(-2 - sc) : X.Lv + 36 * X.zero_blk);
  return base + 6 * X.rho[h];
}
__device__ __forceinline__ double tri1_bcast(double v, int l) {
  return __hiloint2double(__builtin_amdgcn_readlane(__double2hiint(v), l), __builtin_amdgcn_readlane(__double2loint(v), l));
}
constexpr int tri1_low(int i, int j) { return i * (i - 1) / 2 + j; }
__device__ __forceinline__ bool tri1_chol6(const double *__restrict__ sd, int lane, double (&Ls)[15], double (&invd)[6]) {
  Row6 row = load_row(&sd[6 * (lane < 5 ? lane : 5)]);
  bool ok = true;
#pragma unroll
  for (int j = 0; j < 6; ++j) {
    const double d = tri1_bcast(row.v[j], j);
    if (!(d > 0.0)) ok = false;
    const double inv = rsqrt_nr(d);
    invd[j] = inv;
    row.v[j] *= inv;
#pragma unroll
    for (int k = 0; k < 6; ++k)
      if (k > j) {
        const double lkj = tri1_bcast(row.v[j], k);
        Ls[tri1_low(k, j)] = lkj;
        row.v[k] = fma(-row.v[j], lkj, row.v[k]);
      }
  }
  return ok;
}
__device__ __forceinline__ Row6 tri1_trsm_row(const Row6 &u, const double (&Ls)[15], const double (&invd)[6]) {
  Row6 x, w = u;
#pragma unroll
  for (int c = 0; c < 6; ++c) {
    x.v[c] = w.v[c] * invd[c];
#pragma unroll
    for (int c2 = 0; c2 < 6; ++c2) if (c2 > c) w.v[c2] = fma(-x.v[c], Ls[tri1_low(c2, c)], w.v[c2]);
  }
  return x;
}
template <int K>
__device__ __forceinline__ void tri1_step(const Tri1Ctx &X, d4_t (&C)[NJMAX * (NJMAX + 1) / 2], Row6 (&sN)[2], bool &ok_all,
                                          double *__restrict__ W, double *__restrict__ Dt, double *__restrict__ D6,
                                          const int *__restrict__ tsrc, const int *__restrict__ tblk) {
  constexpr int c0 = 6 * K, K0 = c0 >> 4, K1 = (c0 + 5) >> 4;
  const int lane = X.lane, nn = X.nn, q = X.q;
  Row6 s[2] = {sN[0], sN[1]};
  if (K + 1 < X.m) {
#pragma unroll
    for (int h = 0; h < 2; ++h)
      if (X.rv[h] && X.rr[h] >= K + 1) sN[h] = load_row(tri1_src_row(X, tsrc, h, K + 1));
  }
#pragma unroll
  for (int h = 0; h < 2; ++h)
    if (X.rv[h] && X.rr[h] == K && tsrc[K * PM + K] <= -2) {
#pragma unroll
      for (int c = 0; c < 6; ++c) s[h].v[c] += (c == X.rho[h]) ? X.lambda : 0.0;
    }
  if constexpr (K > 0) {
#pragma unroll
    for (int I = 0; I < NJMAX; ++I)
#pragma unroll
      for (int Kt = 0; Kt < NJMAX; ++Kt)
        if ((Kt == K0 || Kt == K1) && Kt <= I && 16 * I + 15 >= c0 && I < X.nJ) {
          const int c = 16 * Kt + nn - c0;
          if (c >= 0 && c < 6) {
#pragma unroll
            for (int r4 = 0; r4 < 4; ++r4) W[(16 * I + q + 4 * r4) * 6 + c] = C[tri1_tile(I, Kt)][r4];
          }
        }
    __builtin_amdgcn_wave_barrier();
#pragma unroll
    for (int h = 0; h < 2; ++h)
// ... 80 lines not shown
  if (!task_runs(P, dsc.task)) return;
  Tri1Ctx X;
  X.Hblk = Hblk; X.Lv = Lv; X.zero_blk = P.zero_blk;
  X.m = dsc.m; X.n = 6 * dsc.m; X.nJ = (X.n + 15) >> 4;
  X.lane = threadIdx.x; X.nn = X.lane & 15; X.q = X.lane >> 4;
  X.lambda = *lambda_p;
  X.tp = P.pp.ptop + (int64_t)dsc.top * 256;
  const int lane = X.lane, n = X.n, nJ = X.nJ;
#pragma unroll
  for (int e = 0; e < PM * PM / 64; ++e) {
    tsrc[lane + 64 * e] = P.pp.ptri_src[(int64_t)pn * PM * PM + lane + 64 * e];
    tblk[lane + 64 * e] = P.pp.ptri_blk[(int64_t)pn * PM * PM + lane + 64 * e];
  }
  for (int e = lane; e < NJMAX * 256; e += 64) {
    const int i = (e >> 4) & 15, j = e & 15, J = e >> 8;
    Dt[e] = (i == j && 16 * J + i >= n) ? 1.0 : 0.0;
  }
#pragma unroll
  for (int h = 0; h < 2; ++h) {
    const int i = lane + 64 * h;
    X.rv[h] = i < n; X.rpad[h] = i < 16 * nJ && i < TRI1_NR;
    X.rr[h] = i / 6; X.rho[h] = i - 6 * X.rr[h];
  }
  __builtin_amdgcn_wave_barrier();
  d4_t C[NJMAX * (NJMAX + 1) / 2];
#pragma unroll
  for (int p = 0; p < NJMAX * (NJMAX + 1) / 2; ++p) C[p] = d4_t{0.0, 0.0, 0.0, 0.0};
  Row6 sN[2];
#pragma unroll
  for (int h = 0; h < 2; ++h) {
    sN[h] = Row6{{0, 0, 0, 0, 0, 0}};
    if (X.rv[h]) sN[h] = load_row(tri1_src_row(X, tsrc, h, 0));
  }
  bool ok_all = true;
  tri1_steps<0>(X, C, sN, ok_all, W, Dt, D6, tsrc, tblk);
  if (!ok_all && lane == 0) atomicOr(fail_flag, 1);
  __builtin_amdgcn_wave_barrier();
#pragma unroll
  for (int pass = 0; pass < (NJMAX + 3) / 4; ++pass) {
    const int J = 4 * pass + X.q, c = X.nn;
    if (J < nJ) {
      const double *__restrict__ D = &Dt[J * 256];
      double xc[16];
#pragma unroll
      for (int i = 0; i < 16; ++i) xc[i] = (i == c) ? 1.0 : 0.0;
#pragma unroll
      for (int i = 0; i < 16; ++i) {
        xc[i] *= 1.0 / D[i * 17];
#pragma unroll
        for (int i2 = 0; i2 < 16; ++i2) if (i2 > i) xc[i2] = fma(-D[i2 * 16 + i], xc[i], xc[i2]);
      }
#pragma unroll
      for (int i = 0; i < 16; ++i) X.tp[(NLT + J) * 256 + 16 * c + i] = xc[i];
    }
  }
}
__global__ __launch_bounds__(64) __attribute__((amdgpu_waves_per_eu(2, 2))) void k_panel_tri1(DevPlan P, const double *__restrict__ Hblk, double *__restrict__ Lv, int pn0,
                                                   const double *__restrict__ lambda_p, int *__restrict__ fail_flag) {
  tri1_body(P, Hblk, Lv, pn0, lambda_p, fail_flag);
}

__device__ __forceinline__ void ride_item_wave(const DevPlan &P, const double *__restrict__ Hblk, double *__restrict__ Lv,
                                               const double *__restrict__ lambda_p, int item, double *__restrict__ tile) {
  const RideItem it = P.ride_items[item];
  if (P.task_dirty && !P.task_dirty[it.task]) return;
  const int lane = threadIdx.x;
  const int g = lane / 6, r = lane - 6 * g;
  if (lane < 60) {
    Row6 acc = {{0, 0, 0, 0, 0, 0}};
    if (g == 0) acc = it.first ? load_A_row(P, Hblk, it.t, r, *lambda_p) : load_row(Lv + 36 * (int64_t)it.t + 6 * r);
    apply_ops(P, Lv, acc, g, r, it.o0 + g, it.o0 + it.n, 10, tile);
#pragma unroll
    for (int c = 0; c < 6; ++c) tile[6 * lane + c] = acc.v[c];
  }
  __builtin_amdgcn_wave_barrier();
  if (lane < 36) {
    double sum = 0;
#pragma unroll
    for (int q = 0; q < 10; ++q) sum += tile[q * 36 + lane];
    Lv[36 * (int64_t)it.t + lane] = sum;
  }
}

template <bool BYC = false>
__device__ __forceinline__ void panel_rows_body(const DevPlan &P, const double *__restrict__ Hblk, double *__restrict__ Lv, int chunk0,
                                                double *__restrict__ x, int n_chunks, const double *__restrict__ lambda_p, int ride0) {
  if ((int)blockIdx.x >= n_chunks) {
    __shared__ __attribute__((aligned(16))) double ride_tile[360];
    ride_item_wave(P, Hblk, Lv, lambda_p, ride0 + (int)blockIdx.x - n_chunks, ride_tile);
    return;
  }
  const int ci = chunk0 + xcd_contiguous(blockIdx.x, n_chunks);
  const RowChunk rc = P.pp.rchunks[ci];
  const int lane = threadIdx.x, nn = lane & 15, q = lane >> 4;
  int scq[4 * NJMAX];
  if constexpr (BYC) {
    const int *__restrict__ rsq = P.pp.rchunk_src + ((int64_t)(ci - P.pp.rchunk_src0) * 16 + nn) * PANEL_MAX;
#pragma unroll
    for (int e = 0; e < 4 * NJMAX; ++e) scq[e] = rsq[(16 * (e >> 2) + q + 4 * (e & 3)) / 6];
  }
  if (!task_runs(P, rc.task)) return;
  const int m = rc.m;
  const int n = 6 * m, nJ = (n + 15) >> 4;
  const int R6 = rc.R6;
  const int *__restrict__ cols = P.task_cols + rc.cols0;
  const double *__restrict__ tp = P.pp.ptop + (int64_t)rc.top * 256;
  constexpr int RS = ROW_SETS;
  constexpr int NE = 4 * NJMAX;
  int sc[RS][NE], rho[RS];
  int64_t rowoff[RS];
  bool valid[RS], rhs[RS];
#pragma unroll
  for (int u = 0; u < RS; ++u) {
    const int s = rc.s0 + 16 * u + nn;
    valid[u] = s < R6;
    rhs[u] = x != nullptr && s == R6;
    const int br = valid[u] ? s / 6 : 0;
    rho[u] = valid[u] ? s - 6 * br : 0;
    rowoff[u] = (int64_t)(rc.prow0 + br) * PM;
    const int *__restrict__ rs = P.pp.prow_src + rowoff[u];
#pragma unroll
    for (int e = 0; e < NE; ++e) {
      const int c = 16 * (e >> 2) + q + 4 * (e & 3);
      if constexpr (BYC) sc[u][e] = ((valid[u] || rhs[u]) && c < n) ? scq[e] : -1;
      else sc[u][e] = (valid[u] && c < n) ? rs[c / 6] : ((rhs[u] && c < n) ? cols[c / 6] : -1);
    }
  }
  d4_t Y[RS][NJMAX];
#pragma unroll
  for (int u = 0; u < RS; ++u)
#pragma unroll
    for (int e = 0; e < NE; ++e) {
      const int c = 16 * (e >> 2) + q + 4 * (e & 3);
      const int k = c / 6;
      const int code = sc[u][e];
      const double *base = code >= 0 ? Lv + 36 * (int64_t)code : (code <= -2 ? Hblk + 36 * (int64_t)(-2 - code) : Lv + 36 * (int64_t)P.zero_blk);
      if (rhs[u] && c < n) base = x + 6 * (int64_t)code;
      Y[u][e >> 2][e & 3] = base[6 * rho[u] + (c - 6 * k)];
    }
  auto load_tile_row = [&](int J, double (&A)[4 * NJMAX]) {
#pragma unroll
    for (int I = 0; I < NJMAX; ++I)
      if (I < J) {
#pragma unroll
        for (int kc = 0; kc < 4; ++kc) A[4 * I + kc] = tp[((J * (J - 1) / 2 + I) * 4 + kc) * 64 + lane];
      }
#pragma unroll
    for (int kc = 0; kc < 4; ++kc) A[4 * (NJMAX - 1) + kc] = tp[((NLT + J) * 4 + kc) * 64 + lane];
  };
  double Abuf[2][4 * NJMAX];
  load_tile_row(0, Abuf[0]);
#pragma unroll
  for (int J = 0; J < NJMAX; ++J)
    if (J < nJ) {
      double (&A)[4 * NJMAX] = Abuf[J & 1];
      if (J + 1 < nJ) load_tile_row(J + 1, Abuf[(J + 1) & 1]);
#pragma unroll
      for (int u = 0; u < RS; ++u) {
        d4_t acc = Y[u][J];
#pragma unroll
        for (int I = 0; I < J; ++I)
#pragma unroll
          for (int kc = 0; kc < 4; ++kc)
            acc = __builtin_amdgcn_mfma_f64_16x16x4f64(A[4 * I + kc], Y[u][I][kc], acc, 0, 0, 0);
        d4_t z = {0.0, 0.0, 0.0, 0.0};
#pragma unroll
        for (int kc = 0; kc < 4; ++kc) z = __builtin_amdgcn_mfma_f64_16x16x4f64(A[4 * (NJMAX - 1) + kc], acc[kc], z, 0, 0, 0);
        Y[u][J] = z;
      }
    }
#pragma unroll
  for (int u = 0; u < RS; ++u) {
    const int *__restrict__ rb = P.pp.prow_blk + rowoff[u];
    int tt[NE];
#pragma unroll
    for (int e = 0; e < NE; ++e) {
      const int c = 16 * (e >> 2) + q + 4 * (e & 3);
      tt[e] = (valid[u] && c < n) ? rb[c / 6] : -1;
    }
#pragma unroll
    for (int e = 0; e < NE; ++e) {
      const int c = 16 * (e >> 2) + q + 4 * (e & 3);
      if (tt[e] >= 0) Lv[36 * (int64_t)tt[e] + 6 * rho[u] + (c - 6 * (c / 6))] = Y[u][e >> 2][e & 3];
      if (rhs[u] && c < n) x[6 * (int64_t)sc[u][e] + (c - 6 * (c / 6))] = Y[u][e >> 2][e & 3];
    }
  }
}

__global__ __launch_bounds__(64) void k_panel_rows(DevPlan P, const double *__restrict__ Hblk, double *__restrict__ Lv, int chunk0,
                                                   double *__restrict__ x, int n_chunks, const double *__restrict__ lambda_p, int ride0) {
  panel_rows_body<false>(P, Hblk, Lv, chunk0, x, n_chunks, lambda_p, ride0);
}
__global__ __launch_bounds__(64) void k_panel_rows_byc(DevPlan P, const double *__restrict__ Hblk, double *__restrict__ Lv, int chunk0,
                                                       double *__restrict__ x, int n_chunks, const double *__restrict__ lambda_p, int ride0) {
  panel_rows_body<true>(P, Hblk, Lv, chunk0, x, n_chunks, lambda_p, ride0);
}

__global__ __launch_bounds__(64) void k_dist_acc(DevPlan P, const double *__restrict__ Hblk, double *__restrict__ Lv,
                                                 const double *__restrict__ lambda_p) {
  __shared__ __attribute__((aligned(16))) double tile[360];
  const int lane = threadIdx.x, g = lane / 6, r = lane - 6 * g;
  const int64_t q = (int64_t)blockIdx.x * 10 + g;
  const int64_t nq = (int64_t)P.zero_blk - P.top_blk0;
  const bool on = lane < 60 && q < nq;
  Row6 acc = {{0, 0, 0, 0, 0, 0}};
  const int64_t t = P.top_blk0 + (on ? q : 0);
  if (on) {
    const int a = P.asrc[t];
    if (a >= 0) {
      acc = load_row(Hblk + 36 * (int64_t)a + 6 * r);
      if (a < P.nb && P.lambda_rank) {
        const double lambda = *lambda_p;
#pragma unroll
        for (int c = 0; c < 6; ++c) acc.v[c] += (c == r) ? lambda : 0.0;
      }
    }
  }
  apply_ops(P, Lv, acc, g, r, on ? P.own_op0[q] : 0, on ? P.own_op1[q] : 0, 1, tile);
  if (on) store_row(Lv + 36 * t + 6 * r, acc);
}
__global__ __launch_bounds__(64) void k_dist_rhs(DevPlan P, const double *__restrict__ Lv, const double *__restrict__ bvec, double *__restrict__ x,
                                                 const double *__restrict__ bfull) {
  __shared__ double sred[60];
  const int kq = blockIdx.x, k = P.top_col0 + kq;
  const int lane = threadIdx.x, g = lane / 6, r = lane - 6 * g;
  const int64_t e0 = P.own_row0[kq], e1 = P.own_row1[kq];
  double acc = 0;
  if (lane < 60) {
    for (int64_t e = e0 + g; e < e1; e += 40) {
      int bi[4], ci[4];
#pragma unroll
      for (int q = 0; q < 4; ++q) {
        const int64_t ee = e + 10 * q;
        const bool in = ee < e1;
        bi[q] = in ? P.row_blk[ee] : P.zero_blk;
        ci[q] = in ? P.row_col[ee] : 0;
      }
      Row6 l[4], y[4];
#pragma unroll
      for (int q = 0; q < 4; ++q) { l[q] = load_row(Lv + 36 * (int64_t)bi[q] + 6 * r); y[q] = load_row(x + 6 * (int64_t)ci[q]); }
#pragma unroll
      for (int q = 0; q < 4; ++q)
        acc += l[q].v[0] * y[q].v[0] + l[q].v[1] * y[q].v[1] + l[q].v[2] * y[q].v[2] + l[q].v[3] * y[q].v[3] + l[q].v[4] * y[q].v[4] + l[q].v[5] * y[q].v[5];
    }
    sred[lane] = acc;
  }
  __syncthreads();
  if (lane < 6) {
    double sv = P.lambda_rank ? bvec[6 * (int64_t)k + lane] : (bfull ? bvec[6 * (int64_t)k + lane] - bfull[6 * (int64_t)k + lane] : 0.0);
    for (int q = 0; q < 10; ++q) sv -= sred[q * 6 + lane];
    x[6 * (int64_t)k + lane] = sv;
  }
}

void prepare_device_kernels() {
  static std::mutex mu;
  static std::vector<char> done;
  int dev = 0;
  if (hipGetDevice(&dev) != hipSuccess || dev < 0) return;
  std::lock_guard<std::mutex> lock(mu);
  if ((int)done.size() <= dev) done.resize(dev + 1, 0);
  if (done[dev]) return;
  (void)hipFuncSetAttribute(reinterpret_cast<const void *>(&k_chol_leaf<4>), hipFuncAttributeMaxDynamicSharedMemorySize, 160 * 1024);
  done[dev] = 1;
}

struct LevelRange {
  bool nothing_dirty;
  int64_t sf, sn;
  int64_t lf; int n_long;
  int n_acc_wg;
  bool fw_table;
  int col0, n_fwd_wg;
  int64_t g2f; int n_g2;
  int t0, nt, pn0;
  int c0, nc;
};
static LevelRange level_range(const HostSchedule &H, const PartialSweep *ps, int l, bool fwd) {
  LevelRange R{};
  const int64_t a0 = H.acc_ptr[l], am = H.acc_mid[l], a1 = H.acc_ptr[l + 1];
  const int t0f = H.level_ptr[l], ntf = H.level_ptr[l + 1] - t0f;
  const bool panel = H.level_panel[l];
  const int n_g2_full = H.g2_lvl.empty() ? 0 : (int)(H.g2_lvl[l + 1] - H.g2_lvl[l]);
  const int64_t g2_first = H.g2_lvl.empty() ? 0 : H.g2_lvl[l];
  R.fw_table = H.fwg_ptr[l + 1] - H.fwg_ptr[l] != H.level_col_ptr[l + 1] - H.level_col_ptr[l];
  R.col0 = R.fw_table ? -1 - H.fwg_ptr[l] : H.level_col_ptr[l];
  const int n_fwd_full = (fwd && panel) ? (R.fw_table ? H.fwg_ptr[l + 1] - H.fwg_ptr[l] : H.level_col_ptr[l + 1] - H.level_col_ptr[l]) : 0;
  const int ta = ps ? ps->t_lo[l] : 0, tb = ps ? ps->t_hi[l] : -1;
  R.nothing_dirty = ps && tb < ta;
  if (!ps) {
    R.sf = a0; R.sn = am - a0;
    R.lf = am; R.n_long = (int)(a1 - am);
    R.n_fwd_wg = n_fwd_full;
    R.g2f = g2_first; R.n_g2 = n_g2_full;
    R.t0 = t0f; R.nt = ntf;
    if (panel) { R.c0 = H.rchunk_ptr[l]; R.nc = H.rchunk_ptr[l + 1] - H.rchunk_ptr[l]; }
  } else if (R.nothing_dirty) {
    R.sf = a0; R.sn = 0;
    R.lf = am; R.n_long = 0;
    R.n_fwd_wg = 0;
    R.g2f = g2_first; R.n_g2 = 0;
    R.t0 = t0f; R.nt = 0;
    if (panel) { R.c0 = H.rchunk_ptr[l]; R.nc = 0; }
  } else {
    R.sf = ps->s0[ta]; R.sn = ps->s1[tb] - ps->s0[ta];
    R.lf = ps->l0[ta]; R.n_long = (int)(ps->l1[tb] - ps->l0[ta]);
    R.n_fwd_wg = n_fwd_full;
    if (n_fwd_full > 0 && !R.fw_table) { R.col0 = ps->task_ptr[ta]; R.n_fwd_wg = ps->task_ptr[tb + 1] - ps->task_ptr[ta]; }
    if (n_g2_full == 0) { R.g2f = g2_first; R.n_g2 = 0; }
    else { R.g2f = ps->g0[ta]; R.n_g2 = ps->g1[tb] - ps->g0[ta]; }
    R.t0 = ta; R.nt = tb - ta + 1;
    if (panel) { R.c0 = ps->c0[ta]; R.nc = ps->c1[tb] - ps->c0[ta]; }
  }
  R.n_acc_wg = R.n_long > 0 ? (cdiv(R.sn, 10) + 7) & ~7 : cdiv(R.sn, 10);
  R.pn0 = panel ? H.level_pn0[l] + (R.t0 - t0f) : 0;
  return R;
}

void launch_factor(const DevPlan &P, const HostSchedule &H, const double *Hblk, double *Lv, const double *lambda_p,
                   int *fail_flag, hipStream_t s, const double *b, double *x, int phase, const PartialSweep *ps, const double *b_full, LaunchCensus *cz) {
  if (x && phase != PHASE_TOP && !P.task_dirty && !cz) launch_copy_vec(b, x, (int64_t)P.top_col0 * 6, s);
  if (cz) { cz->level_riders.assign((size_t)H.n_levels, 0); cz->level_long.assign((size_t)H.n_levels, 0); cz->level_fwd.assign((size_t)H.n_levels, 0); cz->level_fwtab.assign((size_t)H.n_levels, 0); }
  for (int l = 0; l < H.n_levels; ++l) {
    if (!seg_runs(H, l, phase)) continue;
    const LevelRange R = level_range(H, ps, l, x != nullptr);
    const int grid = R.n_acc_wg + R.n_long + R.n_fwd_wg, grid2 = R.n_g2 + R.n_fwd_wg;
    if (cz) { cz->level_fwd[(size_t)l] = R.n_fwd_wg; cz->level_fwtab[(size_t)l] = (R.fw_table && R.n_fwd_wg > 0) ? 1 : 0; }
    const LaunchForm acc = select_acc(H, l);
    const bool acc_g2 = acc == LF_ACC2_8 || acc == LF_ACC2_4 || acc == LF_ACC2_1;
    if (cz && !acc_g2 && grid > 0) cz->level_long[(size_t)l] = R.n_long;
    if (acc_g2 ? grid2 > 0 : grid > 0)
      switch (acc) {
        case LF_ACC2_8: FGO_LAUNCH_N(cz, acc, grid2, R.n_g2, k_chol_acc2<8>, dim3(grid2), dim3(512), 0, s, P, Hblk, Lv, Lv, R.g2f, R.n_g2, lambda_p, x, R.col0); break;
        case LF_ACC2_4: FGO_LAUNCH_N(cz, acc, grid2, R.n_g2, k_chol_acc2<4>, dim3(grid2), dim3(256), 0, s, P, Hblk, Lv, Lv, R.g2f, R.n_g2, lambda_p, x, R.col0); break;
        case LF_ACC2_1: FGO_LAUNCH_N(cz, acc, grid2, R.n_g2, k_chol_acc2<1>, dim3(grid2), dim3(64), 0, s, P, Hblk, Lv, Lv, R.g2f, R.n_g2, lambda_p, x, R.col0); break;
        case LF_ACC8: FGO_LAUNCH_N(cz, acc, grid, R.sn + R.n_long, k_chol_acc<8>, dim3(grid), dim3(512), 0, s, P, Hblk, Lv, R.sf, R.sn, lambda_p, x, R.n_acc_wg, R.col0, R.n_long, R.lf); break;
        case LF_ACC4: FGO_LAUNCH_N(cz, acc, grid, R.sn + R.n_long, k_chol_acc<4>, dim3(grid), dim3(256), 0, s, P, Hblk, Lv, R.sf, R.sn, lambda_p, x, R.n_acc_wg, R.col0, R.n_long, R.lf); break;
        case LF_ACC2: FGO_LAUNCH_N(cz, acc, grid, R.sn + R.n_long, k_chol_acc<2>, dim3(grid), dim3(128), 0, s, P, Hblk, Lv, R.sf, R.sn, lambda_p, x, R.n_acc_wg, R.col0, R.n_long, R.lf); break;
        default: FGO_LAUNCH_N(cz, LF_ACC1, grid, R.sn + R.n_long, k_chol_acc<1>, dim3(grid), dim3(64), 0, s, P, Hblk, Lv, R.sf, R.sn, lambda_p, x, R.n_acc_wg, R.col0, R.n_long, R.lf); break;
      }
    if (x && H.level_panel[l] && !H.fsplit_ptr.empty() && H.fsplit_ptr[l + 1] > H.fsplit_ptr[l] && !R.nothing_dirty)
      FGO_LAUNCH(cz, LF_FWD_COMBINE, H.fsplit_ptr[l + 1] - H.fsplit_ptr[l], k_fwd_combine, dim3(H.fsplit_ptr[l + 1] - H.fsplit_ptr[l]), dim3(64), 0, s, P, x, H.fsplit_ptr[l]);
    const int t0 = R.t0, nt = R.nt;
    if (H.level_panel[l]) {
      switch (select_tri(H, l)) {
        case LF_TRI1:
          if (nt > 0) FGO_LAUNCH(cz, LF_TRI1, nt, k_panel_tri1, dim3(nt), dim3(64), 0, s, P, Hblk, Lv, R.pn0, lambda_p, fail_flag);
          break;
        case LF_TRI8:
          if (nt > 0) FGO_LAUNCH(cz, LF_TRI8, nt, (k_panel_tri<8>), dim3(nt), dim3(8 * 64), 0, s, P, Hblk, Lv, R.pn0, lambda_p, fail_flag, nt, 0, 0, nt);
          break;
        default: {
          constexpr int TRI_NW = 16;
          const int r0 = H.ride_ptr.empty() ? 0 : H.ride_ptr[2 * l], nr = H.ride_ptr.empty() ? 0 : H.ride_ptr[2 * l + 1] - r0;
          const int ntp = (nr > 0 && P.ride_xcd) ? (nt + 7) & ~7 : nt;
          if (ntp + nr > 0) {
            if (cz) cz->level_riders[(size_t)l] += nr;
            FGO_LAUNCH(cz, LF_TRI16, ntp + (nr + RIDE_PER_WG - 1) / RIDE_PER_WG, (k_panel_tri<TRI_NW>), dim3(ntp + (nr + RIDE_PER_WG - 1) / RIDE_PER_WG), dim3(TRI_NW * 64), 0, s, P, Hblk, Lv, R.pn0, lambda_p, fail_flag, ntp, r0, nr, nt);
          }
        }
      }
      const int q0 = H.ride_ptr.empty() ? 0 : H.ride_ptr[2 * l + 1], nq = H.ride_ptr.empty() ? 0 : H.ride_ptr[2 * l + 2] - q0;
      if (R.nc + nq > 0) {
        if (cz) cz->level_riders[(size_t)l] += nq;
        if (select_rows(H, l) == LF_ROWS_BYC) FGO_LAUNCH(cz, LF_ROWS_BYC, R.nc + nq, k_panel_rows_byc, dim3(R.nc + nq), dim3(64), 0, s, P, Hblk, Lv, R.c0, x, R.nc, lambda_p, q0);
        else FGO_LAUNCH(cz, LF_ROWS, R.nc + nq, k_panel_rows, dim3(R.nc + nq), dim3(64), 0, s, P, Hblk, Lv, R.c0, x, R.nc, lambda_p, q0);
      }
      continue;
    }
    if (nt <= 0) continue;
    const LaunchForm fact = select_fact(H, l);
    switch (fact) {
      case LF_LEAF4: {
        const int lb = H.level_leaf_maxblk[l], lc = H.level_maxtaskcols[l];
        const size_t lds = ((size_t)lb + 1) * 36 * sizeof(double) + (size_t)12 * lc * sizeof(double) + ((size_t)lb + 2 + lc + 2) * sizeof(int) +
                           ((size_t)lb + 2) * sizeof(unsigned short) + (size_t)H.level_leaf_maxops[l] * sizeof(unsigned);
        FGO_LAUNCH(cz, LF_LEAF4, nt, (k_chol_leaf<4>), dim3(nt), dim3(256), lds, s, P, Hblk, Lv, t0, lambda_p, fail_flag, lb, lc, x);
        break;
      }
      case LF_FACT_1_2: FGO_LAUNCH(cz, fact, nt, (k_chol_fact<1, 2>), dim3(nt), dim3(64), 0, s, P, Hblk, Lv, t0, lambda_p, fail_flag); break;
      case LF_FACT_1_3: FGO_LAUNCH(cz, fact, nt, (k_chol_fact<1, 3>), dim3(nt), dim3(64), 0, s, P, Hblk, Lv, t0, lambda_p, fail_flag); break;
      case LF_FACT_4_3: FGO_LAUNCH(cz, fact, nt, (k_chol_fact<4, 3>), dim3(nt), dim3(256), 0, s, P, Hblk, Lv, t0, lambda_p, fail_flag); break;
      case LF_FACT_8_3: FGO_LAUNCH(cz, fact, nt, (k_chol_fact<8, 3>), dim3(nt), dim3(512), 0, s, P, Hblk, Lv, t0, lambda_p, fail_flag); break;
      default: FGO_LAUNCH(cz, LF_FACT_16_2, nt, (k_chol_fact<16, 2>), dim3(nt), dim3(1024), 0, s, P, Hblk, Lv, t0, lambda_p, fail_flag); break;
    }
    if (x && fact != LF_LEAF4) launch_fwd_level(P, H, Lv, x, l, s, cz);
  }
  if (phase == PHASE_DOMAIN && !cz) {
    if (H.n_top_blocks > 0) hipLaunchKernelGGL(k_dist_acc, dim3(cdiv(H.n_top_blocks, 10)), dim3(64), 0, s, P, Hblk, Lv, lambda_p);
    if (x && H.n_top_cols > 0) hipLaunchKernelGGL(k_dist_rhs, dim3(H.n_top_cols), dim3(64), 0, s, P, Lv, b, x, b_full);
  }
}

}
```

### graph_slam_amd/csrc/launch_select.cpp

```cpp
#include "device_plan.hpp"
#include "fgo_internal.hpp"

namespace fgo {

const char *launch_form_name(int form) {
  static const char *const names[LF_COUNT] = {
    "k_chol_acc<8>", "k_chol_acc<4>", "k_chol_acc<2>", "k_chol_acc<1>", "k_chol_acc2<8>", "k_chol_acc2<4>", "k_chol_acc2<1>", "k_fwd_combine",
    "k_panel_tri<16>", "k_panel_tri<8>", "k_panel_tri1", "k_panel_rows", "k_panel_rows_byc", "k_chol_leaf<4>",
    "k_chol_fact<1,2>", "k_chol_fact<1,3>", "k_chol_fact<4,3>", "k_chol_fact<8,3>", "k_chol_fact<16,2>",
    "k_solve_fwd<1>", "k_solve_fwd<4>", "k_solve_fwd<16>", "k_fwd_ext", "k_fwd_tri",
    "k_bwd_chain", "k_bwd_fused", "k_bwd_ext", "k_bwd_tri", "k_solve_bwd<1>", "k_solve_bwd<4>", "k_solve_bwd<8>"};
  return form >= 0 && form < LF_COUNT ? names[form] : "?";
}
LaunchForm select_acc(const HostSchedule &H, int l) {
  const int n_g2_full = H.g2_lvl.empty() ? 0 : (int)(H.g2_lvl[l + 1] - H.g2_lvl[l]);
  if (n_g2_full > 0) {
    static const int g2_narrow = (int)tune("acc2_narrow", 400);
    static const int g2_mid = (int)tune("acc2_mid", 6000);
    return n_g2_full <= g2_narrow ? LF_ACC2_8 : n_g2_full <= g2_mid ? LF_ACC2_4 : LF_ACC2_1;
  }
  const int64_t n = H.acc_ptr[l + 1] - H.acc_ptr[l];
  static const int64_t narrow_max = (int64_t)tune("acc_narrow", 4000);
  static const int64_t acc_wide2 = (int64_t)tune("acc_wide2", 60000);
  static const int64_t acc_mid2 = (int64_t)tune("acc_mid2", 15000);
  static const int acc_wide_split = (int)tune("acc_wide_split", 1);
  if (n <= narrow_max) return LF_ACC8;
  if (n > acc_wide2) return acc_wide_split == 1 ? LF_ACC1 : LF_ACC2;
  return n > acc_mid2 ? LF_ACC2 : LF_ACC4;
}
LaunchForm select_tri(const HostSchedule &H, int l) {
  const int ntf = H.level_ptr[l + 1] - H.level_ptr[l];
  const int tri_wide = tri_wide_panels(H.cus);
  static const int tri1_on = (int)tune("tri1", 1);
  const int tri1_min = (int)tune("tri1_min", 3 * H.cus);
  if (tri1_on && ntf > tri_wide && ntf >= tri1_min) return LF_TRI1;
  return ntf > tri_wide ? LF_TRI8 : LF_TRI16;
}
LaunchForm select_rows(const HostSchedule &H, int l) { return l >= H.rows_byc_level ? LF_ROWS_BYC : LF_ROWS; }
LaunchForm select_fact(const HostSchedule &H, int l) {
  if (!H.level_leaf.empty() && H.level_leaf[l]) return LF_LEAF4;
  static const int h1_2 = (int)tune("fact_h1_2", 20), h1_3 = (int)tune("fact_h1_3", 30), h4 = (int)tune("fact_h4", 120), h8 = (int)tune("fact_h8", 240);
  const bool single = H.level_maxtaskcols[l] == 1;
  const int h = H.level_maxcol[l];
  if (single && h <= h1_2) return LF_FACT_1_2;
  if (single && h <= h1_3) return LF_FACT_1_3;
  return h <= h4 ? LF_FACT_4_3 : h <= h8 ? LF_FACT_8_3 : LF_FACT_16_2;
}
LaunchForm select_fwd(const HostSchedule &H, int l) {
  static const int h1 = (int)tune("fwd_h1", 40), h4 = (int)tune("fwd_h4", 160);
  if (H.level_maxtaskcols[l] == 1 && H.level_maxrow[l] <= h1) return LF_FWD1;
  return H.level_maxrow[l] <= h4 ? LF_FWD4 : LF_FWD16;
}
LaunchForm select_bwd(const HostSchedule &H, int l) {
  if (H.level_panel[l]) {
    static const int bwd_fused_max = (int)tune("bwd_fused", 256);
    return H.level_ptr[l + 1] - H.level_ptr[l] <= bwd_fused_max ? LF_BWD_FUSED : LF_BWD_EXT;
  }
  static const int h1 = (int)tune("bwd_h1", 20), h4 = (int)tune("bwd_h4", 80);
  if (H.level_maxtaskcols[l] == 1 && H.level_maxcol[l] <= h1) return LF_BWD1;
  return H.level_maxcol[l] <= h4 ? LF_BWD4 : LF_BWD8;
}

}
```

### graph_slam_amd/csrc/structure_upload.cpp

```cpp
#include "structure_build.hpp"

namespace fgo {
namespace {

int upload_factor_side(fgo_ctx *c, const VarIndex &V, const Ordering &O, const HostTables &T, HubPlan &hubs, size_t &hub_cap) {
  hipStream_t s = c->stream;
  HIPCHK(c, c->d_pose_col.upload(T.pose_col, s));
  if (V.R > 0) {
    HIPCHK(c, c->d_edge_i.alloc((size_t)T.E_cap)); HIPCHK(c, c->d_edge_j.alloc((size_t)T.E_cap)); HIPCHK(c, c->d_edge_slot.alloc((size_t)T.E_cap));
    HIPCHK(c, c->d_edge_kind.alloc((size_t)T.E_cap)); HIPCHK(c, c->d_he.alloc((size_t)2 * T.E_cap));
    HIPCHK(c, c->d_imu.alloc((size_t)T.NI_cap)); HIPCHK(c, c->d_imu_ids.alloc((size_t)6 * T.NI_cap)); HIPCHK(c, c->d_imu_slot.alloc((size_t)15 * T.NI_cap));
    HIPCHK(c, c->d_imu_list.alloc((size_t)T.NI_cap));
  }
  HIPCHK(c, c->d_edge_i.upload(c->ei, s));
  HIPCHK(c, c->d_edge_j.upload(c->ej, s));
  HIPCHK(c, c->d_edge_slot.upload(T.edge_slot, s));
  HIPCHK(c, c->d_he_ptr.upload(T.he_ptr, s));
  plan_hubs(T.he_ptr, V.NX, 0, hubs);
  hub_cap = hubs.var.size() + (V.R > 0 ? 256 : 0);
  { const int rc = upload_hubs(c, hubs, hub_cap); if (rc) return rc; }
  HIPCHK(c, c->d_he.upload(T.he, s));
  HIPCHK(c, c->d_dup_ptr.upload(T.dup_ptr, s));
  HIPCHK(c, c->d_dup_edges.upload(T.dup_edges, s));
  HIPCHK(c, c->d_dup_slot.upload(T.dup_slot, s));
  c->n_dup_members = (int64_t)T.dup_edges.size();
  HIPCHK(c, c->d_ainv.upload(T.erec, s));
  { const int rc = upload_priors(c, V.NX, T.var_mine); if (rc) return rc; }
  HIPCHK(c, c->d_imu.upload(c->imu_payload, s));
  HIPCHK(c, c->d_imu_ids.upload(c->imu_ids, s));
  HIPCHK(c, c->d_imu_slot.upload(T.imu_slot, s));
  {
    std::vector<int> vk(c->var_kind);
    vk.resize((size_t)V.NX, 5);
    HIPCHK(c, c->d_var_kind.upload(vk, s));
    HIPCHK(c, hipStreamSynchronize(s));
  }
  HIPCHK(c, c->d_edge_kind.upload(c->torder, s));
  HIPCHK(c, c->d_imu_list.upload(T.imu_list, s));
  HIPCHK(c, c->d_pose_group.upload(c->pose_group, s));
  HIPCHK(c, c->d_var_mine.upload(T.var_mine, s));
  HIPCHK(c, c->d_top_ext0.upload(T.top_ext0, s));
  HIPCHK(c, c->d_own_op0.upload(T.own_op0, s));
  HIPCHK(c, c->d_own_op1.upload(T.own_op1, s));
  HIPCHK(c, c->d_top_row0.upload(T.top_row0, s));
  HIPCHK(c, c->d_own_row0.upload(T.own_row0, s));
  HIPCHK(c, c->d_own_row1.upload(T.own_row1, s));
  if (O.dist) HIPCHK(c, c->d_gather.alloc(std::max<size_t>((size_t)V.N * 8, 64)));
  return FGO_OK;
}

int host_schedule(fgo_ctx *c, const Ordering &O) {
  hipStream_t s = c->stream;
  const Symbolic &S = c->S;
  DevPlan &P = c->plan;
  c->sched.world = O.world; c->sched.rank = O.rank; c->sched.seg_group = S.seg_group;
  c->sched.n_top_blocks = S.nnzL - O.top_blk0; c->sched.n_top_cols = O.nb - O.top_col0;
  c->sched.ride_ptr = S.ride_items.empty() ? std::vector<int>() : S.ride_ptr;
  c->sched.g2_lvl = S.g2_lvl;
  if (S.g2_ptr.size() <= 1) c->sched.g2_lvl.clear();
  c->sched.level_panel = S.level_panel; c->sched.pchunk_ptr = S.pchunk_ptr; c->sched.fchunk_ptr = S.fchunk_ptr; c->sched.rchunk_ptr = S.rchunk_ptr;
  if (std::getenv("FGO_NO_PANELS")) std::fill(c->sched.level_panel.begin(), c->sched.level_panel.end(), 0);
  c->sched.level_leaf = S.level_leaf; c->sched.level_leaf_maxblk = S.level_leaf_maxblk; c->sched.level_leaf_maxops = S.level_leaf_maxops;
  if (tune("no_leaf", 0) != 0) std::fill(c->sched.level_leaf.begin(), c->sched.level_leaf.end(), 0);
  c->sched.n_levels = (int)S.level_ptr.size() - 1;
  c->sched.level_ptr = S.level_ptr;
  c->sched.acc_ptr = S.acc_ptr; c->sched.acc_mid = S.acc_mid;
  c->sched.level_pn0.assign(c->sched.n_levels, 0);
  for (int l = 0; l < c->sched.n_levels; ++l)
    if (S.level_panel[l]) {
      c->sched.level_pn0[l] = S.task_panel[S.level_ptr[l]];
      for (int t = S.level_ptr[l]; t < S.level_ptr[l + 1]; ++t)
        if (S.task_panel[t] != c->sched.level_pn0[l] + (t - S.level_ptr[l])) return fail(c, FGO_EINVAL, "internal: panel ids of a level are not consecutive");
    }
  c->sched.level_col_ptr.resize(c->sched.n_levels + 1);
  for (int l = 0; l <= c->sched.n_levels; ++l) c->sched.level_col_ptr[l] = S.task_ptr[S.level_ptr[l]];
  {
    static const int fwd_split = (int)tune("fwd_split", 32);
    std::vector<int> fwg_ci, fwg_ch, fsplit, f0v((size_t)O.nb, 0), fnv((size_t)O.nb, 1);
    c->sched.fwg_ptr.assign((size_t)c->sched.n_levels + 1, 0);
    c->sched.fsplit_ptr.assign((size_t)c->sched.n_levels + 1, 0);
    for (int l = 0; l < c->sched.n_levels; ++l) {
      if (S.level_panel[l])
        for (int t = S.level_ptr[l]; t < S.level_ptr[l + 1]; ++t) {
          const int pn = S.task_panel[t], m = S.task_ptr[t + 1] - S.task_ptr[t];
          for (int q = 0; q < m; ++q) {
            const int ci = S.task_ptr[t] + q;
            const int f0 = S.pcol_fchunk0[S.col_off(pn) + q], fn = S.pcol_fchunkn[S.col_off(pn) + q];
            if (fn <= 1 || O.dist || !fwd_split || fn < fwd_split) { fwg_ci.push_back(ci); fwg_ch.push_back(-1); continue; }
            f0v[(size_t)ci] = f0; fnv[(size_t)ci] = fn; fsplit.push_back(ci);
            for (int x = 0; x < fn; ++x) { fwg_ci.push_back(ci); fwg_ch.push_back(f0 + x); }
          }
        }
      c->sched.fwg_ptr[(size_t)l + 1] = (int)fwg_ci.size();
      c->sched.fsplit_ptr[(size_t)l + 1] = (int)fsplit.size();
    }
    HIPCHK(c, c->d_fwg_ci.upload(fwg_ci, s)); HIPCHK(c, c->d_fwg_ch.upload(fwg_ch, s));
    HIPCHK(c, c->d_fwd_f0.upload(f0v, s)); HIPCHK(c, c->d_fwd_fn.upload(fnv, s));
    HIPCHK(c, c->d_fsplit_ci.upload(fsplit, s));
    HIPCHK(c, hipStreamSynchronize(s));
    P.fwg_ci = c->d_fwg_ci.p; P.fwg_ch = c->d_fwg_ch.p; P.fwd_f0 = c->d_fwd_f0.p; P.fwd_fn = c->d_fwd_fn.p; P.fsplit_ci = c->d_fsplit_ci.p;
  }
  c->sched.level_maxcol.assign(c->sched.n_levels, 0);
  c->sched.level_maxrow.assign(c->sched.n_levels, 0);
  c->sched.level_maxtaskcols.assign(c->sched.n_levels, 0);
  for (int l = 0; l < c->sched.n_levels; ++l)
    for (int t = S.level_ptr[l]; t < S.level_ptr[l + 1]; ++t) {
      c->sched.level_maxtaskcols[l] = std::max(c->sched.level_maxtaskcols[l], S.task_ptr[t + 1] - S.task_ptr[t]);
      for (int q = S.task_ptr[t]; q < S.task_ptr[t + 1]; ++q) {
        const int k = S.task_cols[q];
        c->sched.level_maxcol[l] = std::max(c->sched.level_maxcol[l], (int)(S.colptr[k + 1] - S.colptr[k]));
        c->sched.level_maxrow[l] = std::max(c->sched.level_maxrow[l], (int)(S.rowptr[k + 1] - S.rowptr[k]));
      }
    }
  return FGO_OK;
}

int upload_symbolic(fgo_ctx *c, const Ordering &O, const HostTables &T) {
  hipStream_t s = c->stream;
  Symbolic &S = c->S;
  HIPCHK(c, c->d_colptr.upload(S.colptr, s));
  HIPCHK(c, c->d_rowidx.upload(S.rowidx, s));
  HIPCHK(c, c->d_asrc.upload(T.asrc, s));
  HIPCHK(c, c->d_op_ptr.upload(S.op_ptr, s));
  HIPCHK(c, c->d_op_mid.upload(S.op_mid, s));
  HIPCHK(c, c->d_op_a.upload(S.op_a, s));
  HIPCHK(c, c->d_op_b.upload(S.op_b, s));
  HIPCHK(c, c->d_acc_targets.upload(S.acc_targets, s));
  for (auto &a : S.g2_a) if (a < 0) a = (int)S.nnzL;
  HIPCHK(c, c->d_g2_tgt.upload(S.g2_tgt, s));
  HIPCHK(c, c->d_g2_ptr.upload(S.g2_ptr, s));
  HIPCHK(c, c->d_g2_b.upload(S.g2_b, s));
  HIPCHK(c, c->d_g2_a.upload(S.g2_a, s));
  HIPCHK(c, c->d_ride_items.upload(S.ride_items, s));
  HIPCHK(c, c->d_acc_start.upload(S.acc_start, s));
  {
    std::vector<AccDesc> ad(S.acc_targets.size());
    parallel_ranges((int)ad.size(), 1 << 14, [&](int q0, int q1) {
      for (int q = q0; q < q1; ++q) {
        const int t = S.acc_targets[(size_t)q];
        const int64_t rsv = S.acc_start.empty() ? -1 : S.acc_start[(size_t)q];
        const bool from_h = rsv >= 0 && ((rsv >> 62) & 1);
        const int64_t rs = rsv >= 0 ? (rsv & ~((int64_t)1 << 62)) : -1;
        const bool topb = O.dist && t >= O.top_blk0;
        ad[(size_t)q] = AccDesc{t, (topb || (rs >= 0 && !from_h)) ? -2 : (T.asrc[(size_t)t] >= 0 ? T.asrc[(size_t)t] : -1),
                                (long long)(rs >= 0 ? rs : (topb ? T.top_ext0[(size_t)(t - O.top_blk0)] : S.op_ptr[(size_t)t])), (long long)S.op_mid[(size_t)t]};
      }
    });
    HIPCHK(c, c->d_acc_desc.upload(ad, s));
  }
  return FGO_OK;
}

int partial_sweep_tables(fgo_ctx *c, const VarIndex &V, const Ordering &O, const std::vector<int> &task_level, BuildTimer &tm) {
  hipStream_t s = c->stream;
  const Symbolic &S = c->S;
// ... 86 lines not shown
  HIPCHK(c, c->d_panel_task.upload(S.panel_task, s));
  HIPCHK(c, c->d_ptri_blk.upload(S.ptri_blk, s));
  HIPCHK(c, c->d_prow_ptr.upload(S.prow_ptr, s));
  HIPCHK(c, c->d_prow_idx.upload(S.prow_idx, s));
  HIPCHK(c, c->d_prow_blk.upload(S.prow_blk, s));
  HIPCHK(c, c->d_pchunk_panel.upload(S.pchunk_panel, s));
  HIPCHK(c, c->d_pchunk_row0.upload(S.pchunk_row0, s));
  HIPCHK(c, c->d_pchunk_nrows.upload(S.pchunk_nrows, s));
  HIPCHK(c, c->d_panel_chunk0.upload(S.panel_chunk0, s));
  HIPCHK(c, c->d_row_mid.upload(S.row_mid, s));
  HIPCHK(c, c->d_fchunk_col.upload(S.fchunk_col, s));
  HIPCHK(c, c->d_fchunk_e0.upload(S.fchunk_e0, s));
  HIPCHK(c, c->d_pcol_fchunk0.upload(S.pcol_fchunk0, s));
  HIPCHK(c, c->d_pcol_fchunkn.upload(S.pcol_fchunkn, s));
  HIPCHK(c, c->d_ptri_src.upload(T.ptri_src, s));
  HIPCHK(c, c->d_prow_src.upload(T.prow_src, s));
  HIPCHK(c, c->d_rchunk_panel.upload(S.rchunk_panel, s));
  HIPCHK(c, c->d_rchunk_s0.upload(S.rchunk_s0, s));
  HIPCHK(c, c->d_fpart.alloc(S.fchunk_col.size() * 6));
  HIPCHK(c, c->d_bpart.alloc(S.pchunk_panel.size() * PANEL_MAX * 6));
  return FGO_OK;
}

int upload_descriptors(fgo_ctx *c, const Ordering &O, const HostTables &T, const std::vector<int> &task_level, int &byc_level, int &byc_c0) {
  hipStream_t s = c->stream;
  const Symbolic &S = c->S;
  std::vector<PanelDesc> pd((size_t)S.n_panels);
  int64_t n_tiles = 0;
  for (int pn = 0; pn < S.n_panels; ++pn) {
    const int t = S.panel_task[pn];
    const int rows = S.prow_ptr[pn + 1] - S.prow_ptr[pn];
    const bool has = S.level_panel[task_level[t]];
    pd[pn] = PanelDesc{t, S.task_ptr[t + 1] - S.task_ptr[t], S.task_ptr[t], S.prow_ptr[pn], rows, S.panel_chunk0[pn],
                       (rows + PANEL_ROWS - 1) / PANEL_ROWS, has ? (int)n_tiles : -1};
    if (has) n_tiles += NTILE;
  }
  if (n_tiles > INT32_MAX) return fail(c, FGO_ENOMEM, "operand-tile table too large");
  HIPCHK(c, c->d_ptop.alloc((size_t)n_tiles * PTOP_TILE));
  std::vector<RowChunk> rc(S.rchunk_panel.size());
  for (size_t q = 0; q < rc.size(); ++q) {
    const PanelDesc &d = pd[S.rchunk_panel[q]];
    rc[q] = RowChunk{S.rchunk_panel[q], d.m, S.rchunk_s0[q], 6 * d.nrows, d.prow0, d.cols0, d.top, d.task};
  }
  std::vector<BwdChunk> bc(S.pchunk_panel.size());
  for (size_t q = 0; q < bc.size(); ++q) bc[q] = BwdChunk{S.pchunk_panel[q], pd[S.pchunk_panel[q]].m, S.pchunk_row0[q], S.pchunk_nrows[q]};
  HIPCHK(c, c->d_pdesc.upload(pd, s));
  {
    std::vector<int> order((size_t)S.n_panels);
    for (int pn = 0; pn < S.n_panels; ++pn) order[(size_t)pn] = pn;
    const int mode = (int)tune("tri_lpt", 1);
    if (mode != 0)
      for (size_t l = 0; l + 1 < S.level_ptr.size(); ++l) {
        const int ntf = S.level_ptr[l + 1] - S.level_ptr[l];
        if (!S.level_panel[l] || ntf <= 0) continue;
        const int p0 = S.task_panel[S.level_ptr[l]], p1 = p0 + ntf;
        if (p0 < 0 || p1 > S.n_panels) continue;
        const bool tri1 = select_tri(c->sched, (int)l) == LF_TRI1;
        const bool ascending = mode == 2 || (mode == 1 && tri1);
        if (ascending) std::stable_sort(order.begin() + p0, order.begin() + p1, [&](int a, int b) { return pd[(size_t)a].m < pd[(size_t)b].m; });
        else std::stable_sort(order.begin() + p0, order.begin() + p1, [&](int a, int b) { return pd[(size_t)a].m > pd[(size_t)b].m; });
      }
    HIPCHK(c, c->d_tri_order.upload(order, s));
  }
  {
    const int ntask = (int)S.task_ptr.size() - 1;
    std::vector<LeafDesc> ld((size_t)ntask, LeafDesc{0, 0, 0, 0, 0, 0, 0, 0}), lpt;
    for (size_t l = 0; l + 1 < S.level_ptr.size(); ++l) {
      if (l >= S.level_leaf.size() || !S.level_leaf[l]) continue;
      for (int t = S.level_ptr[l]; t < S.level_ptr[l + 1]; ++t) {
        const int cb = S.task_ptr[t], m = S.task_ptr[t + 1] - cb, k0 = S.task_cols[cb];
        const int64_t base = S.colptr[k0], nblk = S.colptr[k0 + m] - base, ob = S.op_ptr[base];
        ld[(size_t)t] = LeafDesc{t, cb, m, k0, (long long)base, (long long)ob, (int)nblk, (int)(S.op_ptr[base + nblk] - ob)};
      }
    }
    lpt = ld;
    if (tune("leaf_lpt", 1) != 0)
      for (size_t l = 0; l + 1 < S.level_ptr.size(); ++l)
        if (l < S.level_leaf.size() && S.level_leaf[l])
          std::stable_sort(lpt.begin() + S.level_ptr[l], lpt.begin() + S.level_ptr[l + 1], [](const LeafDesc &a, const LeafDesc &b) { return a.nops + 2 * a.nblk > b.nops + 2 * b.nblk; });
    HIPCHK(c, c->d_leaf_desc.upload(ld, s));
    HIPCHK(c, c->d_leaf_lpt.upload(lpt, s));
  }
  HIPCHK(c, c->d_rchunks.upload(rc, s));
  {
    const int thr = (int)tune("rows_byc", 600);
    const int nl = (int)S.rchunk_ptr.size() - 1;
    int l0 = nl;
    while (l0 > 0 && S.rchunk_ptr[l0] - S.rchunk_ptr[l0 - 1] < thr) --l0;
    byc_level = l0 < nl && thr > 0 ? l0 : (1 << 30);
    byc_c0 = byc_level < nl ? S.rchunk_ptr[byc_level] : (int)rc.size();
    std::vector<int> rsrc((rc.size() - (size_t)byc_c0) * 16 * PANEL_MAX, -1);
    for (size_t q = (size_t)byc_c0; q < rc.size(); ++q) {
      const RowChunk &r = rc[q];
      for (int nn = 0; nn < 16; ++nn) {
        const int sr = r.s0 + nn;
        int *dst = rsrc.data() + ((q - (size_t)byc_c0) * 16 + nn) * PANEL_MAX;
        if (sr < r.R6) { const size_t ro = S.row_off(r.prow0 + sr / 6); for (int k = 0; k < r.m; ++k) dst[k] = T.prow_src[ro + k]; }
        else if (sr == r.R6) for (int k = 0; k < r.m; ++k) dst[k] = S.task_cols[r.cols0 + k];
      }
    }
    if (!rsrc.empty()) HIPCHK(c, c->d_rchunk_src.upload(rsrc, s)); else c->d_rchunk_src.release();
  }
  {
    static const int chain_on = (int)tune("bwd_chain", 1);
    static const int chain_max = (int)tune("bwd_chain_max", 64);
    std::vector<ChainItem> items;
    const int nl = (int)S.level_ptr.size() - 1;
    int low = nl, chain_levels = 0;
    static const int chain_dist = (int)tune("bwd_chain_dist", 1);
    if (chain_on && (O.world == 1 || chain_dist) && !std::getenv("FGO_NO_PANELS"))
      for (int l = nl - 1; l >= 1; --l) {
        if (O.world > 1 && S.seg_group[l] != O.world) continue;
        const int nt = S.level_ptr[l + 1] - S.level_ptr[l];
        if (!S.level_panel[l] || nt > chain_max || nt == 0) break;
        const int need = (int)items.size();
        for (int t = S.level_ptr[l]; t < S.level_ptr[l + 1]; ++t) items.push_back(ChainItem{S.task_panel[t], need});
        low = l;
        ++chain_levels;
      }
    if (chain_levels < 2) { items.clear(); low = -1; }
    c->sched.bchain_low = items.empty() ? -1 : low;
    c->sched.bchain_n = (int)items.size();
    HIPCHK(c, c->d_bchain.upload(items, s));
    HIPCHK(c, c->d_bchain_done.alloc(1));
    HIPCHK(c, hipMemsetAsync(c->d_bchain_done.p, 0, sizeof(unsigned), s));
  }
  HIPCHK(c, c->d_bchunks.upload(bc, s));
  HIPCHK(c, hipStreamSynchronize(s));
  return FGO_OK;
}

int alloc_work_buffers(fgo_ctx *c, const VarIndex &V, const PairGraph &G, const Ordering &O, const HostTables &T, size_t hub_cap) {
  hipStream_t s = c->stream;
  const Symbolic &S = c->S;
  const int64_t N = V.N, R = V.R, NX = V.NX;
  const int nb = O.nb, n_lm = V.n_lm;
  const size_t hblocks = (size_t)nb + (size_t)G.noff;
  c->plan.n_hblocks = (int64_t)hblocks;
  for (int i = 0; i < 2; ++i) {
    HIPCHK(c, c->d_poses[i].alloc((size_t)NX * 8));
    if (R > 0) HIPCHK(c, hipMemsetAsync(c->d_poses[i].p + (size_t)N * 8, 0, sizeof(double) * (size_t)R * 8, s));
    HIPCHK(c, c->d_H[i].alloc(hblocks * 36));
    HIPCHK(c, c->d_b[i].alloc(((size_t)nb + (size_t)n_lm) * 6));
    HIPCHK(c, hipMemsetAsync(c->d_H[i].p, 0, sizeof(double) * hblocks * 36, s));
  }
  HIPCHK(c, c->d_x.alloc(((size_t)nb + (size_t)n_lm) * 6));
  HIPCHK(c, c->d_L.alloc(((size_t)S.nnzL + 2 + (size_t)S.n_scratch) * 36));
  HIPCHK(c, hipMemsetAsync(c->d_L.p + (size_t)S.nnzL * 36, 0, sizeof(double) * 36 * (2 + (size_t)S.n_scratch), s));
  {
    static const double ident[36] = {1, 0, 0, 0, 0, 0, 0, 1, 0, 0, 0, 0, 0, 0, 1, 0, 0, 0, 0, 0, 0, 1, 0, 0, 0, 0, 0, 0, 1, 0, 0, 0, 0, 0, 0, 1};
    HIPCHK(c, hipMemcpyAsync(c->d_L.p + ((size_t)S.nnzL + 1) * 36, ident, sizeof(ident), hipMemcpyHostToDevice, s));
  }
  HIPCHK(c, c->d_scal.alloc(8));
  HIPCHK(c, c->d_fail.alloc(1));
  HIPCHK(c, hipMemsetAsync(c->d_fail.p, 0, sizeof(int), s));
  const size_t npart = std::max<size_t>({(size_t)4096, (size_t)((NX * 4 + 255) / 256) + hub_cap + (size_t)T.NI_cap + 64 + (size_t)((n_lm + 255) / 256),
                                         (size_t)2048 + (size_t)((T.NI_cap + 63) / 64) + 64, (size_t)((NX + 255) / 256) + 64});
  HIPCHK(c, c->d_imu_stash.alloc((size_t)T.NI_cap * 150));
  HIPCHK(c, c->d_partial.alloc(npart));
  HIPCHK(c, hipStreamSynchronize(s));
  return FGO_OK;
}

void fill_plan(fgo_ctx *c, const VarIndex &V, const Ordering &O, const HostTables &T, const HubPlan &hubs, int byc_level, int byc_c0, BuildTimer &tm) {
  const Symbolic &S = c->S;
  DevPlan &P = c->plan;
  P.n_poses = V.NX; P.edge_stride = T.E_cap; P.nb = O.nb; P.pose_col = c->d_pose_col.p; P.imu_stash = c->d_imu_stash.p;
  set_factor_plan(c, V.N, V.E, V.NI, hubs, (int64_t)T.dup_ptr.size() - 1);
  P.lin_priors = 1;
  P.zero_offdiag = O.dist ? 1 : 0;
  P.dist = O.dist ? 1 : 0; P.top_col0 = O.top_col0; P.top_blk0 = O.top_blk0;
  P.top_ext0 = c->d_top_ext0.p; P.own_op0 = c->d_own_op0.p; P.own_op1 = c->d_own_op1.p;
  P.top_row0 = c->d_top_row0.p; P.own_row0 = c->d_own_row0.p; P.own_row1 = c->d_own_row1.p;
  P.var_mine = O.dist ? c->d_var_mine.p : nullptr; P.lambda_rank = O.rank == 0 ? 1 : 0;
  P.colptr = c->d_colptr.p; P.rowidx = c->d_rowidx.p; P.asrc = c->d_asrc.p;
  P.zero_blk = (int)S.nnzL;
  P.prof_tri = std::getenv("FGO_TRI_PROF") ? std::atoi(std::getenv("FGO_TRI_PROF")) : 0;
  P.op_ptr = c->d_op_ptr.p; P.op_mid = c->d_op_mid.p; P.op_a = c->d_op_a.p; P.op_b = c->d_op_b.p;
  P.acc_targets = c->d_acc_targets.p;
  P.g2_tgt = c->d_g2_tgt.p; P.g2_ptr = c->d_g2_ptr.p; P.g2_b = c->d_g2_b.p; P.g2_a = c->d_g2_a.p;
  P.task_dirty = nullptr; P.acc_task = c->d_acc_task.p; P.g2_task = c->d_g2_task.p; P.tcol_task = c->d_tcol_task.p;
  P.ride_xcd = (int)tune("ride_xcd", 1);
  P.ride_items = S.ride_items.empty() ? nullptr : c->d_ride_items.p; P.acc_start = S.acc_start.empty() ? nullptr : c->d_acc_start.p; P.acc_desc = c->d_acc_desc.p;
  P.rowptr = c->d_rowptr.p; P.row_blk = c->d_row_blk.p; P.row_col = c->d_row_col.p;
  P.task_ptr = c->d_task_ptr.p; P.task_cols = c->d_task_cols.p;
  P.partial = c->d_partial.p;
  P.pp.task_panel = c->d_task_panel.p; P.pp.panel_task = c->d_panel_task.p; P.pp.ptri_blk = c->d_ptri_blk.p;
  P.pp.prow_ptr = c->d_prow_ptr.p; P.pp.prow_idx = c->d_prow_idx.p; P.pp.prow_blk = c->d_prow_blk.p;
  P.pp.pchunk_panel = c->d_pchunk_panel.p; P.pp.pchunk_row0 = c->d_pchunk_row0.p; P.pp.pchunk_nrows = c->d_pchunk_nrows.p;
  P.pp.panel_chunk0 = c->d_panel_chunk0.p; P.pp.row_mid = c->d_row_mid.p; P.pp.fchunk_col = c->d_fchunk_col.p;
  P.pp.fchunk_e0 = c->d_fchunk_e0.p; P.pp.pcol_fchunk0 = c->d_pcol_fchunk0.p; P.pp.pcol_fchunkn = c->d_pcol_fchunkn.p;
  P.pp.fpart = c->d_fpart.p; P.pp.bpart = c->d_bpart.p; P.pp.ptop = c->d_ptop.p;
  P.pp.rchunk_panel = c->d_rchunk_panel.p; P.pp.rchunk_s0 = c->d_rchunk_s0.p; P.pp.rchunk_src = c->d_rchunk_src.p; P.pp.rchunk_src0 = byc_c0; c->sched.rows_byc_level = c->d_rchunk_src.p ? byc_level : (1 << 30);
  P.pp.ptri_src = c->d_ptri_src.p; P.pp.prow_src = c->d_prow_src.p;
  P.pp.pdesc = c->d_pdesc.p; P.pp.tri_order = c->d_tri_order.p; P.pp.leaf_desc = c->d_leaf_desc.p; P.pp.leaf_lpt = c->d_leaf_lpt.p; P.pp.rchunks = c->d_rchunks.p; P.pp.bchunks = c->d_bchunks.p; P.pp.bchain = c->d_bchain.p; P.pp.bchain_done = c->d_bchain_done.p;
  if (tm.prof)
    for (size_t l = 0; l < S.level_leaf.size(); ++l)
      if (S.level_leaf[l]) {
        std::vector<int64_t> nb_t;
        int64_t cols = 0;
        for (int t = S.level_ptr[l]; t < S.level_ptr[l + 1]; ++t) {
          const int c0 = S.task_ptr[t], m = S.task_ptr[t + 1] - c0;
          nb_t.push_back(S.colptr[S.task_cols[c0] + m] - S.colptr[S.task_cols[c0]]); cols += m;
        }
        std::sort(nb_t.begin(), nb_t.end());
        std::fprintf(stderr, "[fgo build]    leaf level %zu: %zu tasks, %lld columns, blocks per task min %lld / median %lld / p90 %lld / max %d, most ops %d\n", l,
                     nb_t.size(), (long long)cols, (long long)nb_t.front(), (long long)nb_t[nb_t.size() / 2], (long long)nb_t[nb_t.size() * 9 / 10], S.level_leaf_maxblk[l],
                     S.level_leaf_maxops[l]);
      }
}

}

int upload_structure(fgo_ctx *c, const VarIndex &V, const PairGraph &G, const Ordering &O, const HostTables &T, const BaTables &BA, BuildTimer &tm) {
  const Symbolic &S = c->S;
  HubPlan hubs;
  size_t hub_cap = 0;
  int byc_level = 1 << 30, byc_c0 = 0, rc;
  std::vector<int> task_level((size_t)S.task_ptr.size() - 1, 0);
  for (size_t l = 0; l + 1 < S.level_ptr.size(); ++l)
    for (int t = S.level_ptr[l]; t < S.level_ptr[l + 1]; ++t) task_level[t] = (int)l;
  if ((rc = upload_factor_side(c, V, O, T, hubs, hub_cap)) != FGO_OK) return rc;
  if ((rc = host_schedule(c, O)) != FGO_OK) return rc;
  if ((rc = upload_symbolic(c, O, T)) != FGO_OK) return rc;
  claim_L(c);
  if ((rc = partial_sweep_tables(c, V, O, task_level, tm)) != FGO_OK) return rc;
  if ((rc = upload_panel_lists(c, T)) != FGO_OK) return rc;
  if ((rc = upload_descriptors(c, O, T, task_level, byc_level, byc_c0)) != FGO_OK) return rc;
  if ((rc = alloc_work_buffers(c, V, G, O, T, hub_cap)) != FGO_OK) return rc;
  if ((rc = ba_upload(c, V, O, BA)) != FGO_OK) return rc;
  fill_plan(c, V, O, T, hubs, byc_level, byc_c0, tm);
  if (V.R > 0) snapshot_for_growth(c, V, G, O, T, hubs.deg_limit, hub_cap);
  c->built_N = V.N;
  c->cur = 0;
  c->sinv.release();
  c->h_pose_col.clear();
  c->structure_dirty = false;
  c->host_poses_newer = true;
  c->lin_valid = false;
  return FGO_OK;
}

}
```

### include/fgo.h

```cpp
#ifndef FGO_H
#define FGO_H
#include <stddef.h>
#include <stdint.h>

#ifdef __cplusplus
extern "C" {
#endif
#if defined(__GNUC__)
#pragma GCC visibility push(default)
#endif

#define FGO_OK 0
#define FGO_EINVAL (-1)
#define FGO_ENODEV (-2)
#define FGO_ENOMEM (-3)
#define FGO_ESTATE (-4)
#define FGO_ENUM (-5)

#define FGO_TANGENT_G2O 0
#define FGO_TANGENT_GTSAM 1

typedef struct fgo_ctx fgo_ctx;

typedef struct {
// ... 316 lines not shown
                    double *normal_out , double *curvature_out , double *eigenvalues_out ,
                    int32_t *n_neighbours_out , uint8_t *status_out ,
                    int32_t *neighbour_out , int64_t *dist2_out ,
                    int64_t *scatter_out );
double fgo_debug_map_normals_kernel_ms(void);

typedef struct {
  double fx, fy, cx, cy;
  double z_scale;
  double z_min, z_max;
  int splat;
  double radius;
  int max_half;
  double agree_tol;
  uint8_t background[3];
} fgo_map_render_params;
void fgo_map_render_params_default(fgo_map_render_params *p);
#define FGO_MAP_RENDER_TILES 0
#define FGO_MAP_RENDER_GLOBAL 1
typedef struct { int64_t n_valid, n_drawn, n_pixels, n_meas, n_both, n_agree, n_closer, n_through; } fgo_map_render_view;
typedef struct { int64_t n_points, n_nonfinite; int form, tile_rows; } fgo_map_render_result;
int fgo_map_render_batch(int device, int64_t n_points, const double *xyz ,
                         const uint8_t *color , int channels ,
                         int64_t n_views, const double *pose_w7 ,
                         const double *extrinsic7 , const double *view_offset7 ,
                         int width, int height, const fgo_map_render_params *params ,
                         const uint16_t *depth_meas , fgo_map_render_result *result ,
                         fgo_map_render_view *view_out , int32_t *zq_out ,
                         int32_t *index_out , uint8_t *color_out ,
                         double *rt_out );
double fgo_debug_map_render_kernel_ms(void);

int fgo_optimize_gtsam(fgo_ctx *ctx, int max_iters, fgo_stats *stats );
int fgo_isam2_update(fgo_ctx *ctx, double relinearize_threshold, fgo_stats *stats );
int fgo_isam2_reserve(fgo_ctx *ctx, int reserve_variables, int window);
int fgo_set_growth(fgo_ctx *ctx, int reserve_variables, int window);
int fgo_isam2_set_wildfire(fgo_ctx *ctx, double threshold);
int fgo_isam2_reset(fgo_ctx *ctx);
int fgo_isam2_get_state(fgo_ctx *ctx, int64_t id, double theta7[7], double delta6[6]);
double fgo_error(fgo_ctx *ctx);
int fgo_marginal_cov(fgo_ctx *ctx, int64_t id, double *cov36);
int fgo_marginal_cov_many(fgo_ctx *ctx, int64_t n, const int64_t *ids, double *cov36);
int64_t fgo_marginal_cov_all(fgo_ctx *ctx, int64_t cap, int64_t *ids_out, double *cov36_out);
int fgo_marginal_cov_pairs(fgo_ctx *ctx, int64_t n, const int64_t *id_a, const int64_t *id_b, double *cov36);
int fgo_debug_selinv_stats(const fgo_ctx *ctx, double out[7]);
int fgo_debug_selinv_census(const fgo_ctx *ctx, int64_t out[16]);
int fgo_gate_edges_se3(fgo_ctx *ctx, int64_t n, const int64_t *id_a, const int64_t *id_b, const double *meas7,
                       const double *info_ut21, int tangent_order,
                       double *d2_out, double *chi2_out, double *pred_cov36_out);
int fgo_edge_chi2_se3(fgo_ctx *ctx, int64_t first, int64_t n, double *chi2_out);
int fgo_gate_plane_factors(fgo_ctx *ctx, int64_t n, const int64_t *pose_id, const int64_t *plane_id, const double *z_abcd,
                           const double *cov_ut6, double *d2_out, double *chi2_out, double *cos_out, double *resid3_out,
                           double *pred_cov9_out);
int fgo_associate_planes(fgo_ctx *ctx, int64_t pose_id, int64_t k, const double *z_abcd, const double *cov_ut6, int64_t m,
                         const int64_t *plane_ids, double d2_gate, double cos_min, int64_t *match_out, double *best2_out,
                         double *d2_matrix_out);
int fgo_debug_gate_stats(const fgo_ctx *ctx, double out[4]);

int fgo_optimize(fgo_ctx *ctx, int max_iters, fgo_stats *stats );
double fgo_chi2(fgo_ctx *ctx);
int fgo_trace(const fgo_ctx *ctx, double *chi2s, double *lambdas, int cap);

int fgo_linearize(fgo_ctx *ctx, double *chi2_out, double *H_dense, double *b_dense, int64_t *n_free_out);
int fgo_solve_step(fgo_ctx *ctx, double lambda, double *delta_out);
int fgo_bench_phase(fgo_ctx *ctx, int phase, int reps, double *ms_out);
int fgo_get_stats(const fgo_ctx *ctx, fgo_stats *stats);

int64_t fgo_synth_manhattan3d(int64_t n_poses, int lookback, int n_loop, uint64_t seed, double sigma_t,
                              double sigma_q, double *poses_init7, double *poses_true7, int64_t *id_i,
                              int64_t *id_j, double *meas7, double *info_ut21, int64_t max_edges);

typedef int (*fgo_allreduce_fn)(void *user, double *device_buffer, int64_t count);
int fgo_set_shard(fgo_ctx *ctx, int rank, int world);
int fgo_set_allreduce(fgo_ctx *ctx, fgo_allreduce_fn fn, void *user);
int fgo_dist_unique_id(void *id128);
int fgo_dist_init_rccl(fgo_ctx *ctx, const void *id128);
int fgo_debug_partition(int n, int64_t n_pairs, const int *a, const int *b, int world, int *group_out);
int fgo_debug_allreduce(fgo_ctx *ctx, double *host_buffer, int64_t count);
int fgo_shard_range(int64_t n, int rank, int world, int64_t *lo, int64_t *hi);
int fgo_debug_read_scratch(fgo_ctx *ctx, double *out, int64_t count);
int fgo_debug_read_system(fgo_ctx *ctx, double *H, double *b, double *chi2);
int fgo_debug_read_reduced(fgo_ctx *ctx, double lambda, double *H_dense, double *b_dense, int64_t *n_out);
int fgo_debug_solve_fused(fgo_ctx *ctx, double lambda, double *delta_out);
int fgo_debug_launch_census(fgo_ctx *ctx, int fused, int64_t *launches, int64_t *workgroups, int64_t *items, int form_cap, int *level_riders,
                            int *level_long, int level_cap, int *chain2, char *names, int names_cap);
int fgo_debug_isam_last(fgo_ctx *ctx, int *info5, int *level_lo, int *level_hi, int *level_ntask, int *level_fwd, int *level_fwtab, int level_cap,
                        int *task_level,
                        unsigned char *task_dirty, unsigned char *task_run, int task_cap, int *var_task, unsigned char *var_chg,
                        double *var_delta, int64_t var_cap);
int fgo_debug_linearize_census(fgo_ctx *ctx, int64_t out[12]);

#if defined(__GNUC__)
#pragma GCC visibility pop
#endif
#ifdef __cplusplus
}
#endif
#endif
```

Before: 197.7 iterations/s.

## Fuse panel row-update phase into 16-wave panel triangle kernel for small panels

For panel levels that use the 16-wave triangle kernel and the by-column row kernel, and where each panel has at most a tunable number of row chunks (default 4), the row-chunk update now runs inside the triangle kernel. It reads the inverted triangle tiles straight from LDS instead of launching a separate rows kernel that reloads them from global memory. This removes one launch per such level and the global round-trip of the operand tiles. In exchange it serialises the row work onto the panel's 16 waves and adds LDS writes and scheduling barriers. A debug API to read back the factor is also added for verification.

```diff
diff --git a/graph_slam_amd/__init__.py b/graph_slam_amd/__init__.py
--- a/graph_slam_amd/__init__.py
+++ b/graph_slam_amd/__init__.py
@@ -265,6 +265,8 @@
     lib.fgo_debug_read_system.argtypes = [C.c_void_p, dp, dp, dp]
     lib.fgo_debug_read_reduced.argtypes = [C.c_void_p, C.c_double, dp, dp, i64p]
     lib.fgo_debug_solve_fused.argtypes = [C.c_void_p, C.c_double, dp]
+    if hasattr(lib, "fgo_debug_read_factor"):
+        lib.fgo_debug_read_factor.argtypes = [C.c_void_p, dp, C.c_int64, i64p]
     lib.fgo_debug_launch_census.argtypes = [C.c_void_p, C.c_int, i64p, i64p, i64p, C.c_int, C.POINTER(C.c_int), C.POINTER(C.c_int), C.c_int,
                                             C.POINTER(C.c_int), C.c_char_p, C.c_int]
     lib.fgo_debug_isam_last.argtypes = [C.c_void_p] + [C.POINTER(C.c_int)] * 6 + [C.c_int,
@@ -1478,6 +1480,13 @@
         self._chk(lib.fgo_debug_solve_fused(self._h, lam, _dp(d)))
         return d
 
+    def read_factor(self):
+        n = C.c_int64()
+        self._chk(lib.fgo_debug_read_factor(self._h, None, 0, C.byref(n)))
+        L = np.zeros((n.value, 6, 6))
+        self._chk(lib.fgo_debug_read_factor(self._h, _dp(L), n.value, None))
+        return L
+
     def launch_census(self, fused=True):
         ip = C.POINTER(C.c_int)
         names = C.create_string_buffer(4096)
diff --git a/graph_slam_amd/csrc/device_plan.hpp b/graph_slam_amd/csrc/device_plan.hpp
--- a/graph_slam_amd/csrc/device_plan.hpp
+++ b/graph_slam_amd/csrc/device_plan.hpp
@@ -56,6 +56,7 @@
   const int *rchunk_panel, *rchunk_s0;
   const int *rchunk_src;
   int rchunk_src0;
+  const int *panel_rchunk0;
   const int *ptri_src, *prow_src;
   double *ptop;
   double *fpart;
@@ -204,6 +205,8 @@
   std::vector<int> level_leaf_maxblk, level_leaf_maxops;
   std::vector<char> level_panel;
   int rows_byc_level = 1 << 30;
+  std::vector<int> level_maxrchunks;
+  int tri_rows_cap = 0;
   std::vector<int> level_pn0;
   std::vector<int> level_col_ptr;
   std::vector<int> fwg_ptr;
@@ -230,6 +233,7 @@
   LF_FWD_COMBINE,
   LF_TRI16, LF_TRI8, LF_TRI1,
   LF_ROWS, LF_ROWS_BYC,
+  LF_TRI16_ROWS,
   LF_LEAF4,
   LF_FACT_1_2, LF_FACT_1_3, LF_FACT_4_3, LF_FACT_8_3, LF_FACT_16_2,
   LF_FWD1, LF_FWD4, LF_FWD16,
@@ -250,6 +254,7 @@
 LaunchForm select_acc(const HostSchedule &H, int l);
 LaunchForm select_tri(const HostSchedule &H, int l);
 LaunchForm select_rows(const HostSchedule &H, int l);
+bool select_tri_rows(const HostSchedule &H, int l);
 LaunchForm select_fact(const HostSchedule &H, int l);
 LaunchForm select_fwd(const HostSchedule &H, int l);
 LaunchForm select_bwd(const HostSchedule &H, int l);
diff --git a/graph_slam_amd/csrc/fgo_ctx.hpp b/graph_slam_amd/csrc/fgo_ctx.hpp
--- a/graph_slam_amd/csrc/fgo_ctx.hpp
+++ b/graph_slam_amd/csrc/fgo_ctx.hpp
@@ -101,7 +101,7 @@
   fgo::DevBuf<int> d_hub_list, d_hub_slice, d_hubm;
   fgo::DevBuf<double> d_hub_part;
   fgo::DevBuf<fgo::PanelDesc> d_pdesc;
-  fgo::DevBuf<int> d_tri_order, d_rchunk_src;
+  fgo::DevBuf<int> d_tri_order, d_rchunk_src, d_panel_rchunk0;
   fgo::DevBuf<fgo::LeafDesc> d_leaf_desc, d_leaf_lpt;
   fgo::DevBuf<fgo::AccDesc> d_acc_desc;
   fgo::DevBuf<fgo::RowChunk> d_rchunks;
diff --git a/graph_slam_amd/csrc/fgo_inspect.cpp b/graph_slam_amd/csrc/fgo_inspect.cpp
--- a/graph_slam_amd/csrc/fgo_inspect.cpp
+++ b/graph_slam_amd/csrc/fgo_inspect.cpp
@@ -137,6 +137,19 @@
 int fgo_solve_step(fgo_ctx *c, double lambda, double *delta_out) try { return solve_once(c, lambda, delta_out, false, "fgo_solve_step"); } FGO_CATCH_INT(c)
 int fgo_debug_solve_fused(fgo_ctx *c, double lambda, double *delta_out) try { return solve_once(c, lambda, delta_out, true, "fgo_debug_solve_fused"); } FGO_CATCH_INT(c)
 
+int fgo_debug_read_factor(fgo_ctx *c, double *L, int64_t cap_blocks, int64_t *n_blocks_out) try {
+  if (!c || cap_blocks < 0) return FGO_EINVAL;
+  (void)hipSetDevice(c->cfg.device);
+  if (c->structure_dirty || !c->d_L.p) return fail(c, FGO_ESTATE, "fgo_debug_read_factor: no factorisation has run on the current structure");
+  const int64_t nnz = c->S.nnzL;
+  if (n_blocks_out) *n_blocks_out = nnz;
+  if (!L) return FGO_OK;
+  if (cap_blocks < nnz || (size_t)nnz * 36 > c->d_L.n) return fail(c, FGO_EINVAL, "fgo_debug_read_factor: buffer too small");
+  HIPCHK(c, hipStreamSynchronize(c->stream));
+  HIPCHK(c, hipMemcpy(L, c->d_L.p, sizeof(double) * 36 * (size_t)nnz, hipMemcpyDeviceToHost));
+  return FGO_OK;
+} FGO_CATCH_INT(c)
+
 int fgo_debug_launch_census(fgo_ctx *c, int fused, int64_t *launches, int64_t *workgroups, int64_t *items, int form_cap, int *level_riders, int *level_long,
                             int level_cap, int *chain2, char *names, int names_cap) try {
   if (!c || form_cap < 0 || level_cap < 0 || names_cap < 0) return FGO_EINVAL;
diff --git a/graph_slam_amd/csrc/fgo_internal.hpp b/graph_slam_amd/csrc/fgo_internal.hpp
--- a/graph_slam_amd/csrc/fgo_internal.hpp
+++ b/graph_slam_amd/csrc/fgo_internal.hpp
@@ -34,7 +34,7 @@
   }();
   return nthreads;
 }
-inline double tune(const char *key, double dflt) {
+inline const std::unordered_map<std::string, double> &tune_table() {
   static const std::unordered_map<std::string, double> *tab = [] {
     auto *m = new std::unordered_map<std::string, double>();
     if (const char *e = std::getenv("FGO_TUNE")) {
@@ -51,9 +51,13 @@
     }
     return m;
   }();
-  const auto it = tab->find(key);
-  return it == tab->end() ? dflt : it->second;
-}
+  return *tab;
+}
+inline double tune(const char *key, double dflt) {
+  const auto it = tune_table().find(key);
+  return it == tune_table().end() ? dflt : it->second;
+}
+inline bool tune_is_set(const char *key) { return tune_table().count(key) != 0; }
 class HostPool {
  public:
   static HostPool &get() {
diff --git a/graph_slam_amd/csrc/kernels_factor.hip b/graph_slam_amd/csrc/kernels_factor.hip
--- a/graph_slam_amd/csrc/kernels_factor.hip
+++ b/graph_slam_amd/csrc/kernels_factor.hip
@@ -516,12 +516,18 @@
   }
 }
 
-template <int NW>
-__global__ __launch_bounds__(NW * 64) void k_panel_tri(DevPlan P, const double *__restrict__ Hblk, double *__restrict__ Lv, int pn0,
-                                                    const double *__restrict__ lambda_p, int *__restrict__ fail_flag, int n_pn, int ride0, int n_ride, int n_real) {
+__device__ __forceinline__ void rows_chunk_codes(const DevPlan &P, int ci, int nn, int q, int (&scq)[4 * NJMAX]);
+template <bool BYC, bool LDSA>
+__device__ __forceinline__ void panel_rows_chunk(const DevPlan &P, const double *__restrict__ Hblk, double *__restrict__ Lv, const RowChunk &rc,
+                                                 const int (&scq)[4 * NJMAX], double *__restrict__ x, const double *__restrict__ tp, int lane);
+template <int NW, bool ROWS>
+__device__ __forceinline__ void panel_tri_body(const DevPlan &P, const double *__restrict__ Hblk, double *__restrict__ Lv, int pn0,
+                                               const double *__restrict__ lambda_p, int *__restrict__ fail_flag, int n_pn, int ride0, int n_ride, int n_real,
+                                               double *__restrict__ x) {
+  static_assert(!ROWS || (NW == 16 && ROW_SETS == 1 && NTILE * PTOP_TILE <= 16 * 360), "row phase: 16 waves, the operand tiles fit the rider scratch");
   __shared__ __attribute__((aligned(16))) double T[PM * (PM + 1) / 2 * 36];
+  __shared__ __attribute__((aligned(16))) double ride_smem[NW == 16 ? 16 * 360 : 2];
   if (NW == 16) {
-    __shared__ __attribute__((aligned(16))) double ride_smem[NW == 16 ? 16 * 360 : 2];
     if ((int)blockIdx.x >= n_pn) {
       const int nwg = (int)gridDim.x - n_pn;
       ride_items16(P, Hblk, Lv, lambda_p, ride0, n_ride, P.ride_xcd ? xcd_contiguous((int)blockIdx.x - n_pn, nwg) : (int)blockIdx.x - n_pn, ride_smem);
@@ -676,7 +682,9 @@
     for (int e = e0; e < (nJ * (nJ - 1) / 2) * 256; e += estep) {
       const int tile = e >> 8, kc = (e >> 6) & 3, l = e & 63;
       const int J = PAIR_A[tile] + 1, I = PAIR_B[tile];
-      tp[e] = -Ls(16 * J + (l & 15), 16 * I + 4 * kc + (l >> 4));
+      const double v = -Ls(16 * J + (l & 15), 16 * I + 4 * kc + (l >> 4));
+      tp[e] = v;
+      if constexpr (ROWS) ride_smem[e] = v;
     }
   };
   auto invert = [&]() {
@@ -697,7 +705,10 @@
         for (int i2 = 0; i2 < 16; ++i2) if (i2 > i) xc[i2] = fma(-D[i2 * 16 + i], xc[i], xc[i2]);
       }
 #pragma unroll
-      for (int i = 0; i < 16; ++i) tp[(NLT + J) * 256 + 16 * c + i] = xc[i];
+      for (int i = 0; i < 16; ++i) {
+        tp[(NLT + J) * 256 + 16 * c + i] = xc[i];
+        if constexpr (ROWS) ride_smem[(NLT + J) * 256 + 16 * c + i] = xc[i];
+      }
     }
   };
   if (NW < 16) copy_out(gid, NW * 10, (int)threadIdx.x, NW * 64);
@@ -706,6 +717,29 @@
   if (NW < 16 || wave < 2) invert();
   else copy_out(gid - 20, (NW - 2) * 10, (int)threadIdx.x - 128, (NW - 2) * 64);
   if (stamp && threadIdx.x == 0) { stamp[3] = __builtin_readcyclecounter(); stamp[4] = wall_clock64(); }
+  if constexpr (ROWS) {
+    const int nrc = (6 * dsc.nrows + 16) >> 4;
+    const int rc0 = P.pp.panel_rchunk0[pn];
+    __syncthreads();
+    for (int qc = wave; qc < nrc; qc += NW) {
+      const RowChunk rc{pn, m, 16 * qc, 6 * dsc.nrows, dsc.prow0, dsc.cols0, dsc.top, dsc.task};
+      int ln = lane;
+      asm volatile("" : "+v"(ln));
+      int scq[4 * NJMAX];
+      rows_chunk_codes(P, rc0 + qc, ln & 15, ln >> 4, scq);
+      panel_rows_chunk<true, true>(P, Hblk, Lv, rc, scq, x, ride_smem, ln);
+    }
+  }
+}
+template <int NW>
+__global__ __launch_bounds__(NW * 64) void k_panel_tri(DevPlan P, const double *__restrict__ Hblk, double *__restrict__ Lv, int pn0,
+                                                    const double *__restrict__ lambda_p, int *__restrict__ fail_flag, int n_pn, int ride0, int n_ride, int n_real) {
+  panel_tri_body<NW, false>(P, Hblk, Lv, pn0, lambda_p, fail_flag, n_pn, ride0, n_ride, n_real, nullptr);
+}
+__global__ __launch_bounds__(16 * 64) void k_panel_tri_rows(DevPlan P, const double *__restrict__ Hblk, double *__restrict__ Lv, int pn0,
+                                                            const double *__restrict__ lambda_p, int *__restrict__ fail_flag, int n_pn, int ride0, int n_ride, int n_real,
+                                                            double *__restrict__ x) {
+  panel_tri_body<16, true>(P, Hblk, Lv, pn0, lambda_p, fail_flag, n_pn, ride0, n_ride, n_real, x);
 }
 
 constexpr int tri1_tile(int I, int K) { return I * (I + 1) / 2 + K; }
@@ -952,29 +986,19 @@
   }
 }
 
-template <bool BYC = false>
-__device__ __forceinline__ void panel_rows_body(const DevPlan &P, const double *__restrict__ Hblk, double *__restrict__ Lv, int chunk0,
-                                                double *__restrict__ x, int n_chunks, const double *__restrict__ lambda_p, int ride0) {
-  if ((int)blockIdx.x >= n_chunks) {
-    __shared__ __attribute__((aligned(16))) double ride_tile[360];
-    ride_item_wave(P, Hblk, Lv, lambda_p, ride0 + (int)blockIdx.x - n_chunks, ride_tile);
-    return;
-  }
-  const int ci = chunk0 + xcd_contiguous(blockIdx.x, n_chunks);
-  const RowChunk rc = P.pp.rchunks[ci];
-  const int lane = threadIdx.x, nn = lane & 15, q = lane >> 4;
-  int scq[4 * NJMAX];
-  if constexpr (BYC) {
-    const int *__restrict__ rsq = P.pp.rchunk_src + ((int64_t)(ci - P.pp.rchunk_src0) * 16 + nn) * PANEL_MAX;
-#pragma unroll
-    for (int e = 0; e < 4 * NJMAX; ++e) scq[e] = rsq[(16 * (e >> 2) + q + 4 * (e & 3)) / 6];
-  }
-  if (!task_runs(P, rc.task)) return;
+__device__ __forceinline__ void rows_chunk_codes(const DevPlan &P, int ci, int nn, int q, int (&scq)[4 * NJMAX]) {
+  const int *__restrict__ rsq = P.pp.rchunk_src + ((int64_t)(ci - P.pp.rchunk_src0) * 16 + nn) * PANEL_MAX;
+#pragma unroll
+  for (int e = 0; e < 4 * NJMAX; ++e) scq[e] = rsq[(16 * (e >> 2) + q + 4 * (e & 3)) / 6];
+}
+template <bool BYC, bool LDSA>
+__device__ __forceinline__ void panel_rows_chunk(const DevPlan &P, const double *__restrict__ Hblk, double *__restrict__ Lv, const RowChunk &rc,
+                                                 const int (&scq)[4 * NJMAX], double *__restrict__ x, const double *__restrict__ tp, int lane) {
+  const int nn = lane & 15, q = lane >> 4;
   const int m = rc.m;
   const int n = 6 * m, nJ = (n + 15) >> 4;
   const int R6 = rc.R6;
   const int *__restrict__ cols = P.task_cols + rc.cols0;
-  const double *__restrict__ tp = P.pp.ptop + (int64_t)rc.top * 256;
   constexpr int RS = ROW_SETS;
   constexpr int NE = 4 * NJMAX;
   int sc[RS][NE], rho[RS];
@@ -1007,6 +1031,7 @@
       const double *base = code >= 0 ? Lv + 36 * (int64_t)code : (code <= -2 ? Hblk + 36 * (int64_t)(-2 - code) : Lv + 36 * (int64_t)P.zero_blk);
       if (rhs[u] && c < n) base = x + 6 * (int64_t)code;
       Y[u][e >> 2][e & 3] = base[6 * rho[u] + (c - 6 * k)];
+      if constexpr (LDSA) { if ((e & 7) == 7) __builtin_amdgcn_sched_barrier(0); }
     }
   auto load_tile_row = [&](int J, double (&A)[4 * NJMAX]) {
 #pragma unroll
@@ -1019,12 +1044,12 @@
     for (int kc = 0; kc < 4; ++kc) A[4 * (NJMAX - 1) + kc] = tp[((NLT + J) * 4 + kc) * 64 + lane];
   };
   double Abuf[2][4 * NJMAX];
-  load_tile_row(0, Abuf[0]);
+  if constexpr (!LDSA) load_tile_row(0, Abuf[0]);
 #pragma unroll
   for (int J = 0; J < NJMAX; ++J)
     if (J < nJ) {
       double (&A)[4 * NJMAX] = Abuf[J & 1];
-      if (J + 1 < nJ) load_tile_row(J + 1, Abuf[(J + 1) & 1]);
+      if constexpr (!LDSA) { if (J + 1 < nJ) load_tile_row(J + 1, Abuf[(J + 1) & 1]); }
 #pragma unroll
       for (int u = 0; u < RS; ++u) {
         d4_t acc = Y[u][J];
@@ -1032,29 +1057,62 @@
         for (int I = 0; I < J; ++I)
 #pragma unroll
           for (int kc = 0; kc < 4; ++kc)
-            acc = __builtin_amdgcn_mfma_f64_16x16x4f64(A[4 * I + kc], Y[u][I][kc], acc, 0, 0, 0);
+            acc = __builtin_amdgcn_mfma_f64_16x16x4f64(LDSA ? tp[((J * (J - 1) / 2 + I) * 4 + kc) * 64 + lane] : A[4 * I + kc], Y[u][I][kc], acc, 0, 0, 0);
         d4_t z = {0.0, 0.0, 0.0, 0.0};
 #pragma unroll
-        for (int kc = 0; kc < 4; ++kc) z = __builtin_amdgcn_mfma_f64_16x16x4f64(A[4 * (NJMAX - 1) + kc], acc[kc], z, 0, 0, 0);
+        for (int kc = 0; kc < 4; ++kc)
+          z = __builtin_amdgcn_mfma_f64_16x16x4f64(LDSA ? tp[((NLT + J) * 4 + kc) * 64 + lane] : A[4 * (NJMAX - 1) + kc], acc[kc], z, 0, 0, 0);
         Y[u][J] = z;
       }
     }
+  int ls = lane;
+  if constexpr (LDSA) asm volatile("" : "+v"(ls));
+  const int nns = ls & 15, qs = ls >> 4;
 #pragma unroll
   for (int u = 0; u < RS; ++u) {
-    const int *__restrict__ rb = P.pp.prow_blk + rowoff[u];
+    const int s = rc.s0 + 16 * u + nns;
+    const bool valid_s = s < R6, rhs_s = x != nullptr && s == R6;
+    const int br = valid_s ? s / 6 : 0, rho_s = valid_s ? s - 6 * br : 0;
+    const int *__restrict__ rb = P.pp.prow_blk + (int64_t)(rc.prow0 + br) * PM;
     int tt[NE];
 #pragma unroll
     for (int e = 0; e < NE; ++e) {
-      const int c = 16 * (e >> 2) + q + 4 * (e & 3);
-      tt[e] = (valid[u] && c < n) ? rb[c / 6] : -1;
+      const int c = 16 * (e >> 2) + qs + 4 * (e & 3);
+      tt[e] = (valid_s && c < n) ? rb[c / 6] : -1;
     }
 #pragma unroll
     for (int e = 0; e < NE; ++e) {
-      const int c = 16 * (e >> 2) + q + 4 * (e & 3);
-      if (tt[e] >= 0) Lv[36 * (int64_t)tt[e] + 6 * rho[u] + (c - 6 * (c / 6))] = Y[u][e >> 2][e & 3];
-      if (rhs[u] && c < n) x[6 * (int64_t)sc[u][e] + (c - 6 * (c / 6))] = Y[u][e >> 2][e & 3];
-    }
-  }
+      const int c = 16 * (e >> 2) + qs + 4 * (e & 3);
+      if (tt[e] >= 0) Lv[36 * (int64_t)tt[e] + 6 * rho_s + (c - 6 * (c / 6))] = Y[u][e >> 2][e & 3];
+      if constexpr (!LDSA) { if (rhs_s && c < n) x[6 * (int64_t)sc[u][e] + (c - 6 * (c / 6))] = Y[u][e >> 2][e & 3]; }
+      if constexpr (LDSA) { if ((e & 7) == 7) __builtin_amdgcn_sched_barrier(0); }
+    }
+    if constexpr (LDSA) {
+      if (rhs_s) {
+#pragma unroll
+        for (int e = 0; e < NE; ++e) {
+          const int c = 16 * (e >> 2) + qs + 4 * (e & 3);
+          if (c < n) x[6 * (int64_t)cols[c / 6] + (c - 6 * (c / 6))] = Y[u][e >> 2][e & 3];
+        }
+      }
+    }
+  }
+}
+template <bool BYC = false>
+__device__ __forceinline__ void panel_rows_body(const DevPlan &P, const double *__restrict__ Hblk, double *__restrict__ Lv, int chunk0,
+                                                double *__restrict__ x, int n_chunks, const double *__restrict__ lambda_p, int ride0) {
+  if ((int)blockIdx.x >= n_chunks) {
+    __shared__ __attribute__((aligned(16))) double ride_tile[360];
+    ride_item_wave(P, Hblk, Lv, lambda_p, ride0 + (int)blockIdx.x - n_chunks, ride_tile);
+    return;
+  }
+  const int ci = chunk0 + xcd_contiguous(blockIdx.x, n_chunks);
+  const RowChunk rc = P.pp.rchunks[ci];
+  const int lane = threadIdx.x;
+  int scq[4 * NJMAX];
+  if constexpr (BYC) rows_chunk_codes(P, ci, lane & 15, lane >> 4, scq);
+  if (!task_runs(P, rc.task)) return;
+  panel_rows_chunk<BYC, false>(P, Hblk, Lv, rc, scq, x, P.pp.ptop + (int64_t)rc.top * 256, lane);
 }
 
 __global__ __launch_bounds__(64) void k_panel_rows(DevPlan P, const double *__restrict__ Hblk, double *__restrict__ Lv, int chunk0,
@@ -1213,6 +1271,7 @@
       FGO_LAUNCH(cz, LF_FWD_COMBINE, H.fsplit_ptr[l + 1] - H.fsplit_ptr[l], k_fwd_combine, dim3(H.fsplit_ptr[l + 1] - H.fsplit_ptr[l]), dim3(64), 0, s, P, x, H.fsplit_ptr[l]);
     const int t0 = R.t0, nt = R.nt;
     if (H.level_panel[l]) {
+      const bool tri_rows = select_tri_rows(H, l);
       switch (select_tri(H, l)) {
         case LF_TRI1:
           if (nt > 0) FGO_LAUNCH(cz, LF_TRI1, nt, k_panel_tri1, dim3(nt), dim3(64), 0, s, P, Hblk, Lv, R.pn0, lambda_p, fail_flag);
@@ -1226,15 +1285,22 @@
           const int ntp = (nr > 0 && P.ride_xcd) ? (nt + 7) & ~7 : nt;
           if (ntp + nr > 0) {
             if (cz) cz->level_riders[(size_t)l] += nr;
-            FGO_LAUNCH(cz, LF_TRI16, ntp + (nr + RIDE_PER_WG - 1) / RIDE_PER_WG, (k_panel_tri<TRI_NW>), dim3(ntp + (nr + RIDE_PER_WG - 1) / RIDE_PER_WG), dim3(TRI_NW * 64), 0, s, P, Hblk, Lv, R.pn0, lambda_p, fail_flag, ntp, r0, nr, nt);
+            const int tgrid = ntp + (nr + RIDE_PER_WG - 1) / RIDE_PER_WG;
+            if (tri_rows && R.nc > 0) {
+              if (cz) cz->add(LF_TRI16_ROWS, R.nc);
+              FGO_LAUNCH(cz, LF_TRI16, tgrid, k_panel_tri_rows, dim3(tgrid), dim3(TRI_NW * 64), 0, s, P, Hblk, Lv, R.pn0, lambda_p, fail_flag, ntp, r0, nr, nt, x);
+            } else {
+              FGO_LAUNCH(cz, LF_TRI16, tgrid, (k_panel_tri<TRI_NW>), dim3(tgrid), dim3(TRI_NW * 64), 0, s, P, Hblk, Lv, R.pn0, lambda_p, fail_flag, ntp, r0, nr, nt);
+            }
           }
         }
       }
       const int q0 = H.ride_ptr.empty() ? 0 : H.ride_ptr[2 * l + 1], nq = H.ride_ptr.empty() ? 0 : H.ride_ptr[2 * l + 2] - q0;
-      if (R.nc + nq > 0) {
+      const int n_row = tri_rows ? 0 : R.nc;
+      if (n_row + nq > 0) {
         if (cz) cz->level_riders[(size_t)l] += nq;
-        if (select_rows(H, l) == LF_ROWS_BYC) FGO_LAUNCH(cz, LF_ROWS_BYC, R.nc + nq, k_panel_rows_byc, dim3(R.nc + nq), dim3(64), 0, s, P, Hblk, Lv, R.c0, x, R.nc, lambda_p, q0);
-        else FGO_LAUNCH(cz, LF_ROWS, R.nc + nq, k_panel_rows, dim3(R.nc + nq), dim3(64), 0, s, P, Hblk, Lv, R.c0, x, R.nc, lambda_p, q0);
+        if (select_rows(H, l) == LF_ROWS_BYC) FGO_LAUNCH(cz, LF_ROWS_BYC, n_row + nq, k_panel_rows_byc, dim3(n_row + nq), dim3(64), 0, s, P, Hblk, Lv, R.c0, x, n_row, lambda_p, q0);
+        else FGO_LAUNCH(cz, LF_ROWS, n_row + nq, k_panel_rows, dim3(n_row + nq), dim3(64), 0, s, P, Hblk, Lv, R.c0, x, n_row, lambda_p, q0);
       }
       continue;
     }
diff --git a/graph_slam_amd/csrc/launch_select.cpp b/graph_slam_amd/csrc/launch_select.cpp
--- a/graph_slam_amd/csrc/launch_select.cpp
+++ b/graph_slam_amd/csrc/launch_select.cpp
@@ -6,7 +6,7 @@
 const char *launch_form_name(int form) {
   static const char *const names[LF_COUNT] = {
     "k_chol_acc<8>", "k_chol_acc<4>", "k_chol_acc<2>", "k_chol_acc<1>", "k_chol_acc2<8>", "k_chol_acc2<4>", "k_chol_acc2<1>", "k_fwd_combine",
-    "k_panel_tri<16>", "k_panel_tri<8>", "k_panel_tri1", "k_panel_rows", "k_panel_rows_byc", "k_chol_leaf<4>",
+    "k_panel_tri<16>", "k_panel_tri<8>", "k_panel_tri1", "k_panel_rows", "k_panel_rows_byc", "k_panel_tri<16>+rows", "k_chol_leaf<4>",
     "k_chol_fact<1,2>", "k_chol_fact<1,3>", "k_chol_fact<4,3>", "k_chol_fact<8,3>", "k_chol_fact<16,2>",
     "k_solve_fwd<1>", "k_solve_fwd<4>", "k_solve_fwd<16>", "k_fwd_ext", "k_fwd_tri",
     "k_bwd_chain", "k_bwd_fused", "k_bwd_ext", "k_bwd_tri", "k_solve_bwd<1>", "k_solve_bwd<4>", "k_solve_bwd<8>"};
@@ -37,6 +37,11 @@
   return ntf > tri_wide ? LF_TRI8 : LF_TRI16;
 }
 LaunchForm select_rows(const HostSchedule &H, int l) { return l >= H.rows_byc_level ? LF_ROWS_BYC : LF_ROWS; }
+bool select_tri_rows(const HostSchedule &H, int l) {
+  const int cap = H.tri_rows_cap;
+  if (cap <= 0 || !H.level_panel[l] || (size_t)l >= H.level_maxrchunks.size()) return false;
+  return select_tri(H, l) == LF_TRI16 && select_rows(H, l) == LF_ROWS_BYC && H.level_maxrchunks[l] <= cap;
+}
 LaunchForm select_fact(const HostSchedule &H, int l) {
   if (!H.level_leaf.empty() && H.level_leaf[l]) return LF_LEAF4;
   static const int h1_2 = (int)tune("fact_h1_2", 20), h1_3 = (int)tune("fact_h1_3", 30), h4 = (int)tune("fact_h4", 120), h8 = (int)tune("fact_h8", 240);
diff --git a/graph_slam_amd/csrc/structure_upload.cpp b/graph_slam_amd/csrc/structure_upload.cpp
--- a/graph_slam_amd/csrc/structure_upload.cpp
+++ b/graph_slam_amd/csrc/structure_upload.cpp
@@ -71,6 +71,16 @@
       c->sched.level_pn0[l] = S.task_panel[S.level_ptr[l]];
       for (int t = S.level_ptr[l]; t < S.level_ptr[l + 1]; ++t)
         if (S.task_panel[t] != c->sched.level_pn0[l] + (t - S.level_ptr[l])) return fail(c, FGO_EINVAL, "internal: panel ids of a level are not consecutive");
+    }
+  {
+    const char *e = std::getenv("FGO_TRI_ROWS");
+    c->sched.tri_rows_cap = e ? std::atoi(e) : (tune_is_set("rows_byc") ? 0 : (int)tune("tri_rows", 4));
+  }
+  c->sched.level_maxrchunks.assign(c->sched.n_levels, 0);
+  for (int l = 0; l < c->sched.n_levels; ++l)
+    for (int q = S.rchunk_ptr[l], run = 0; q < S.rchunk_ptr[l + 1]; ++q) {
+      run = (q > S.rchunk_ptr[l] && S.rchunk_panel[q] == S.rchunk_panel[q - 1]) ? run + 1 : 1;
+      c->sched.level_maxrchunks[l] = std::max(c->sched.level_maxrchunks[l], run);
     }
   c->sched.level_col_ptr.resize(c->sched.n_levels + 1);
   for (int l = 0; l <= c->sched.n_levels; ++l) c->sched.level_col_ptr[l] = S.task_ptr[S.level_ptr[l]];
@@ -323,6 +333,11 @@
     HIPCHK(c, c->d_leaf_lpt.upload(lpt, s));
   }
   HIPCHK(c, c->d_rchunks.upload(rc, s));
+  {
+    std::vector<int> first((size_t)S.n_panels, 0);
+    for (size_t q = rc.size(); q-- > 0;) first[(size_t)S.rchunk_panel[q]] = (int)q;
+    HIPCHK(c, c->d_panel_rchunk0.upload(first, s));
+  }
   {
     const int thr = (int)tune("rows_byc", 600);
     const int nl = (int)S.rchunk_ptr.size() - 1;
@@ -432,7 +447,7 @@
   P.pp.panel_chunk0 = c->d_panel_chunk0.p; P.pp.row_mid = c->d_row_mid.p; P.pp.fchunk_col = c->d_fchunk_col.p;
   P.pp.fchunk_e0 = c->d_fchunk_e0.p; P.pp.pcol_fchunk0 = c->d_pcol_fchunk0.p; P.pp.pcol_fchunkn = c->d_pcol_fchunkn.p;
   P.pp.fpart = c->d_fpart.p; P.pp.bpart = c->d_bpart.p; P.pp.ptop = c->d_ptop.p;
-  P.pp.rchunk_panel = c->d_rchunk_panel.p; P.pp.rchunk_s0 = c->d_rchunk_s0.p; P.pp.rchunk_src = c->d_rchunk_src.p; P.pp.rchunk_src0 = byc_c0; c->sched.rows_byc_level = c->d_rchunk_src.p ? byc_level : (1 << 30);
+  P.pp.rchunk_panel = c->d_rchunk_panel.p; P.pp.rchunk_s0 = c->d_rchunk_s0.p; P.pp.rchunk_src = c->d_rchunk_src.p; P.pp.panel_rchunk0 = c->d_panel_rchunk0.p; P.pp.rchunk_src0 = byc_c0; c->sched.rows_byc_level = c->d_rchunk_src.p ? byc_level : (1 << 30);
   P.pp.ptri_src = c->d_ptri_src.p; P.pp.prow_src = c->d_prow_src.p;
   P.pp.pdesc = c->d_pdesc.p; P.pp.tri_order = c->d_tri_order.p; P.pp.leaf_desc = c->d_leaf_desc.p; P.pp.leaf_lpt = c->d_leaf_lpt.p; P.pp.rchunks = c->d_rchunks.p; P.pp.bchunks = c->d_bchunks.p; P.pp.bchain = c->d_bchain.p; P.pp.bchain_done = c->d_bchain_done.p;
   if (tm.prof)
diff --git a/include/fgo.h b/include/fgo.h
--- a/include/fgo.h
+++ b/include/fgo.h
@@ -422,6 +422,7 @@
 int fgo_debug_read_system(fgo_ctx *ctx, double *H, double *b, double *chi2);
 int fgo_debug_read_reduced(fgo_ctx *ctx, double lambda, double *H_dense, double *b_dense, int64_t *n_out);
 int fgo_debug_solve_fused(fgo_ctx *ctx, double lambda, double *delta_out);
+int fgo_debug_read_factor(fgo_ctx *ctx, double *L, int64_t cap_blocks, int64_t *n_blocks_out);
 int fgo_debug_launch_census(fgo_ctx *ctx, int fused, int64_t *launches, int64_t *workgroups, int64_t *items, int form_cap, int *level_riders,
                             int *level_long, int level_cap, int *chain2, char *names, int names_cap);
 int fgo_debug_isam_last(fgo_ctx *ctx, int *info5, int *level_lo, int *level_hi, int *level_ntask, int *level_fwd, int *level_fwtab, int level_cap,
```

Result: no change. 197.6 iterations/s (median of 4 runs) (-0.0%).
